# Kuhlman-Lab/ThermoMPNN

Hardware: AMD Instinct MI355X
Metric: mutant ddG preds/sec (SSM, L=256, K=48) (higher is better)
Workload: dtype f32 (per-edge matmuls: f16x2 split on the 16-bit matrix cores, 22 significant bits, fp32 accumulate); 1 GPU; BASELINE configs[1] x 64: 64 synthetic L=256 proteins per GPU (K=48, h=128), full 20xL SSM each, inputs resident in HBM; proteins_per_gpu=64, L=256, K=48, h=128, unit_counted=mutant ddG predictions, weights=synthetic_state_dict(seed=0), parallelism=proteins sharded x1

## Files before the change

### thermompnn_amd/csrc/tmpnn_api.hip

```cpp
#include <stdarg.h>
#include <stdio.h>
#include <stdlib.h>
#include <string.h>

#include <map>
#include <new>
#include <string>
#include <vector>

#include "tmpnn_internal.h"
#include "tmpnn_head_body.h"
#include "../../include/tmpnn_debug.h"

static thread_local char g_err[512] = "";

int tm_set_error(int code, const char *fmt, ...) {
    va_list ap;
    va_start(ap, fmt);
    vsnprintf(g_err, sizeof(g_err), fmt, ap);
    va_end(ap);
    return code;
}
int tm_check_launch(const char *what) {
    hipError_t e = hipGetLastError();
    if (e != hipSuccess) return tm_set_error(TMPNN_E_LAUNCH, "%s: %s", what, hipGetErrorString(e));
    return TMPNN_OK;
}

struct ProfRec { const char *name; hipEvent_t start, stop; };
static bool g_prof_on = false;
static bool g_prof_open = false;
static std::string g_prof_only;
static std::vector<ProfRec> g_prof;
static std::vector<hipEvent_t> g_event_pool;

static hipEvent_t prof_event() {
    if (!g_event_pool.empty()) { hipEvent_t e = g_event_pool.back(); g_event_pool.pop_back(); return e; }
    hipEvent_t e = nullptr;
    if (hipEventCreate(&e) != hipSuccess) return nullptr;
    return e;
}
void tm_prof_begin(const char *name, hipStream_t st) {
    g_prof_open = false;
    if (!g_prof_on || (!g_prof_only.empty() && g_prof_only != name)) return;
    ProfRec r{name, prof_event(), prof_event()};
    if (!r.start || !r.stop) return;
    (void)hipEventRecord(r.start, st);
    g_prof.push_back(r);
    g_prof_open = true;
}
void tm_prof_end(hipStream_t st) {
    if (!g_prof_open) return;
    (void)hipEventRecord(g_prof.back().stop, st);
    g_prof_open = false;
}

extern "C" int tmpnn_profile_select(const char *name) {
    g_prof_only = name ? name : "";
    return TMPNN_OK;
}

extern "C" int tmpnn_profile_enable(int on) {
    for (auto &r : g_prof) { g_event_pool.push_back(r.start); g_event_pool.push_back(r.stop); }
    g_prof.clear();
    g_prof_on = on != 0;
    return TMPNN_OK;
}

extern "C" int tmpnn_profile_fetch(const char **names, double *total_ms, int64_t *launches, int capacity) {
    if (capacity < 0 || (capacity > 0 && (!names || !total_ms || !launches)))
        return tm_set_error(TMPNN_E_INVALID, "profile_fetch: bad arguments");
    std::vector<const char *> order;
    std::map<std::string, std::pair<double, int64_t>> agg;
    for (auto &r : g_prof) {
        if (hipEventSynchronize(r.stop) != hipSuccess) return tm_set_error(TMPNN_E_LAUNCH, "profile_fetch: event sync failed");
        float ms = 0.f;
        if (hipEventElapsedTime(&ms, r.start, r.stop) != hipSuccess) return tm_set_error(TMPNN_E_LAUNCH, "profile_fetch: elapsed failed");
        auto it = agg.find(r.name);
        if (it == agg.end()) { order.push_back(r.name); agg[r.name] = {ms, 1}; }
        else { it->second.first += ms; it->second.second += 1; }
    }
    int n = 0;
    for (const char *nm : order) {
        if (n >= capacity) break;
        names[n] = nm; total_ms[n] = agg[nm].first; launches[n] = agg[nm].second;
        ++n;
    }
    for (auto &r : g_prof) { g_event_pool.push_back(r.start); g_event_pool.push_back(r.stop); }
    g_prof.clear();
    return n;
}
int tm_num_cus() {
    static int cache[64] = {0};
    int dev = 0;
    if (hipGetDevice(&dev) != hipSuccess || dev < 0 || dev >= 64) return 256;
    if (cache[dev] == 0) {
        int n = 0;
        if (hipDeviceGetAttribute(&n, hipDeviceAttributeMultiprocessorCount, dev) != hipSuccess || n <= 0) n = 256;
        cache[dev] = n;
    }
    return cache[dev];
}

static int parse_mode(const char *e) {
    if (e == nullptr || e[0] == 0 || strcmp(e, "f16x2") == 0) return (int)TM_MM_F16X2;
    if (strcmp(e, "bf16x3") == 0) return (int)TM_MM_BF16X3;
    if (strcmp(e, "fp32") == 0) return (int)TM_MM_FP32;
    return -1;
}
static const char *mode_name(int m) { return m == TM_MM_F16X2 ? "f16x2" : m == TM_MM_BF16X3 ? "bf16x3" : "fp32"; }
static int default_mode() {
    static const int v = parse_mode(getenv("TMPNN_PRECISION"));
    return v;
}
extern "C" const char *tmpnn_matmul_mode(void) { return mode_name(default_mode() < 0 ? (int)TM_MM_F16X2 : default_mode()); }
extern "C" const char *tmpnn_weights_precision(const tmpnn_weights_t *w) { return w ? mode_name(w->mode) : nullptr; }

extern "C" int tmpnn_status_error(int32_t status) {
    if (status == 0) return TMPNN_OK;
    if (status & TMPNN_STATUS_MAXLEN)
        return tm_set_error(TMPNN_E_INVALID, "a protein is longer than the max_len passed to the call (its neighbour rows were left empty)");
    if (status & TMPNN_STATUS_RANGE)
        return tm_set_error(TMPNN_E_RANGE, "non-finite ddG / log-probability: an operand left the fp16 range of the f16x2 "
                                           "matrix-core path (|x| >= 65504); use precision \"bf16x3\" (full fp32 range)");
    if (status & TMPNN_STATUS_SELFTEST)
        return tm_set_error(TMPNN_E_UNSUPPORTED, "device self-test failed: this libtmpnn.so was built with flags under which the f16x2 "
                                                 "GELU does not propagate NaN (fp16 overflow would go undetected) or the code-object "
                                                 "ABI differs from v5 (persistent tile loops would stride wrongly); rebuild with "
                                                 "python -m thermompnn_amd.build");
    return tm_set_error(TMPNN_E_INVALID, "unknown status bits 0x%x", (unsigned)status);
}

extern "C" int tmpnn_selftest(int32_t *status, tmpnn_stream_t stream) {
    if (!status) return tm_set_error(TMPNN_E_INVALID, "selftest: null status word");
    return launch_selftest(status, (hipStream_t)stream);
}

extern "C" int tmpnn_version(void) { return TMPNN_VERSION; }
extern "C" const char *tmpnn_last_error(void) { return g_err; }

struct TensorSpec { std::string name; int64_t numel; };

static const std::vector<TensorSpec> &tensor_table() {
    static std::vector<TensorSpec> t;
    if (!t.empty()) return t;
    auto add = [&](const std::string &n, int64_t e) { t.push_back({n, e}); };
    const int H = TMPNN_HID;
    add("features.embeddings.linear.weight", 16 * 66);
    add("features.embeddings.linear.bias", 16);
    add("features.edge_embedding.weight", H * 416);
    add("features.norm_edges.weight", H);
    add("features.norm_edges.bias", H);
    add("W_e.weight", H * H);
    add("W_e.bias", H);
    add("W_s.weight", TMPNN_VOCAB * H);
    auto layer = [&](const std::string &p, int num_in, bool edge) {
        const char *norms[3] = {"norm1", "norm2", "norm3"};
        for (int i = 0; i < (edge ? 3 : 2); ++i) { add(p + "." + norms[i] + ".weight", H); add(p + "." + norms[i] + ".bias", H); }
        add(p + ".W1.weight", (int64_t)H * (H + num_in)); add(p + ".W1.bias", H);
        add(p + ".W2.weight", H * H); add(p + ".W2.bias", H);
        add(p + ".W3.weight", H * H); add(p + ".W3.bias", H);
        if (edge) {
            add(p + ".W11.weight", (int64_t)H * (H + num_in)); add(p + ".W11.bias", H);
            add(p + ".W12.weight", H * H); add(p + ".W12.bias", H);
            add(p + ".W13.weight", H * H); add(p + ".W13.bias", H);
        }
        add(p + ".dense.W_in.weight", 4 * H * H); add(p + ".dense.W_in.bias", 4 * H);
        add(p + ".dense.W_out.weight", 4 * H * H); add(p + ".dense.W_out.bias", H);
    };
    for (int i = 0; i < 3; ++i) layer("encoder_layers." + std::to_string(i), 2 * H, true);
    for (int i = 0; i < 3; ++i) layer("decoder_layers." + std::to_string(i), 3 * H, false);
    add("W_out.weight", TMPNN_VOCAB * H);
    add("W_out.bias", TMPNN_VOCAB);
    add("light_attention.feature_convolution.weight", 384 * 384 * 9);
    add("light_attention.feature_convolution.bias", 384);
    add("light_attention.attention_convolution.weight", 384 * 384 * 9);
    add("light_attention.attention_convolution.bias", 384);
    add("both_out.1.weight", 64 * 384); add("both_out.1.bias", 64);
    add("both_out.3.weight", 32 * 64); add("both_out.3.bias", 32);
    add("both_out.5.weight", TMPNN_VOCAB * 32); add("both_out.5.bias", TMPNN_VOCAB);
    add("ddg_out.weight", 1); add("ddg_out.bias", 1);
    return t;
}

extern "C" int tmpnn_num_tensors(void) { return (int)tensor_table().size(); }
extern "C" const char *tmpnn_tensor_name(int i) {
    const auto &t = tensor_table();
    return (i < 0 || i >= (int)t.size()) ? nullptr : t[i].name.c_str();
}
extern "C" int64_t tmpnn_tensor_numel(int i) {
    const auto &t = tensor_table();
    return (i < 0 || i >= (int)t.size()) ? -1 : t[i].numel;
}

static const size_t POS_TABLE_FLOATS = 66 * TMPNN_HID, SEQ_TABLE_FLOATS = TMPNN_VOCAB * TMPNN_HID,
                    CONV_CENTER_FLOATS = 384 * 384;
static size_t packed_bytes_for(int mode) {
    return (POS_TABLE_FLOATS + 3 * SEQ_TABLE_FLOATS + CONV_CENTER_FLOATS) * sizeof(float) +
           (mode == TM_MM_F16X2 ? (size_t)TM_N_IMG * TM_WIMG_BYTES : 0);
}
extern "C" size_t tmpnn_weights_packed_bytes(void) { return packed_bytes_for(TM_MM_F16X2); }
extern "C" size_t tmpnn_weights_packed_bytes_p(const char *precision) {
    const int mode = precision ? parse_mode(precision) : default_mode();
    return mode < 0 ? 0 : packed_bytes_for(mode);
}

extern "C" int tmpnn_weights_create(tmpnn_weights_t **out, const float *const *tensors, int n_tensors, void *packed,
                                    size_t packed_bytes, tmpnn_stream_t stream) {
    return tmpnn_weights_create_p(out, tensors, n_tensors, packed, packed_bytes, nullptr, stream);
}

extern "C" int tmpnn_weights_create_p(tmpnn_weights_t **out, const float *const *tensors, int n_tensors, void *packed,
                                      size_t packed_bytes, const char *precision, tmpnn_stream_t stream) {
    const int mode = precision ? parse_mode(precision) : default_mode();
    if (mode < 0)
        return tm_set_error(TMPNN_E_INVALID, "weights_create: unknown precision '%s' (f16x2 | bf16x3 | fp32)",
                            precision ? precision : getenv("TMPNN_PRECISION"));
    if (!out || !tensors || !packed) return tm_set_error(TMPNN_E_INVALID, "weights_create: null argument");
    if (tensor_table().size() != TMPNN_N_TENSORS) return tm_set_error(TMPNN_E_INVALID, "internal tensor table size");
    if (n_tensors != TMPNN_N_MPNN_TENSORS && n_tensors != TMPNN_N_TENSORS)
        return tm_set_error(TMPNN_E_INVALID, "weights_create: n_tensors must be %d or %d, got %d", TMPNN_N_MPNN_TENSORS,
                            TMPNN_N_TENSORS, n_tensors);
    if (packed_bytes < packed_bytes_for(mode))
        return tm_set_error(TMPNN_E_WORKSPACE, "weights_create: packed buffer %zu < %zu bytes", packed_bytes,
                            packed_bytes_for(mode));
    if (((uintptr_t)packed & 15) != 0) return tm_set_error(TMPNN_E_INVALID, "weights_create: packed buffer must be 16-byte aligned");
    for (int i = 0; i < n_tensors; ++i)
        if (!tensors[i] || ((uintptr_t)tensors[i] & 15) != 0)
            return tm_set_error(TMPNN_E_INVALID, "weights_create: tensor %d (%s) is null or not 16-byte aligned", i,
                                tmpnn_tensor_name(i));
    tmpnn_weights *w = new (std::nothrow) tmpnn_weights();
    if (!w) return tm_set_error(TMPNN_E_INVALID, "weights_create: host allocation failed");
    memset(w, 0, sizeof(*w));
    w->n_tensors = n_tensors;
    w->mode = mode;
    std::map<std::string, const float *> by_name;
    for (int i = 0; i < n_tensors; ++i) { w->t[i] = tensors[i]; by_name[tensor_table()[i].name] = tensors[i]; }
    auto get = [&](const std::string &n) -> const float * {
        auto it = by_name.find(n);
        return it == by_name.end() ? nullptr : it->second;
    };
    w->pos_w = get("features.embeddings.linear.weight");
    w->pos_b = get("features.embeddings.linear.bias");
    w->edge_w = get("features.edge_embedding.weight");
    w->norm_edges_w = get("features.norm_edges.weight");
    w->norm_edges_b = get("features.norm_edges.bias");
    w->We_w = get("W_e.weight");
    w->We_b = get("W_e.bias");
    w->Ws_w = get("W_s.weight");
    auto node = [&](const std::string &p) {
        return NodeW{get(p + "W3.weight"), get(p + "W3.bias"), get(p + "norm1.weight"), get(p + "norm1.bias"),
                     get(p + "dense.W_in.weight"), get(p + "dense.W_in.bias"), get(p + "dense.W_out.weight"), get(p + "dense.W_out.bias"),
                     get(p + "norm2.weight"), get(p + "norm2.bias"), {}};
    };
    auto proj = [](const float *W, int ld, int c_off, const float *b) {
        return NodeProj{ProjSpec{W, ld, b, W + c_off, ld, nullptr, nullptr, nullptr}, {}};
    };
    for (int l = 0; l < 3; ++l) {
        const std::string p = "encoder_layers." + std::to_string(l) + ".";
        const float *W1 = get(p + "W1.weight"), *W11 = get(p + "W11.weight");
        EncW &e = w->enc[l];
        e.node = node(p);
        e.msg = MsgW{W1 + 128, 384, get(p + "W2.weight"), get(p + "W2.bias"), false, {}};
        e.edge = EdgeW{W11 + 128, get(p + "W12.weight"), get(p + "W12.bias"), get(p + "W13.weight"), get(p + "W13.bias"),
                       get(p + "norm3.weight"), get(p + "norm3.bias"), {}};
        e.msg_proj = proj(W1, 384, 256, get(p + "W1.bias"));
        e.edge_proj = proj(W11, 384, 256, get(p + "W11.bias"));
        const std::string d = "decoder_layers." + std::to_string(l) + ".";
        const float *D1 = get(d + "W1.weight");
        DecW &c = w->dec[l];
        c.node = node(d);
        c.msg = MsgW{D1 + 128, 512, get(d + "W2.weight"), get(d + "W2.bias"), true, {}};
        c.msg_proj = proj(D1, 512, 384, get(d + "W1.bias"));
    }
    w->Wout_w = get("W_out.weight");
    w->Wout_b = get("W_out.bias");
    if (n_tensors == TMPNN_N_TENSORS) {
        w->conv_w = get("light_attention.feature_convolution.weight");
        w->conv_b = get("light_attention.feature_convolution.bias");
        const char *idx[3] = {"1", "3", "5"};
        for (int i = 0; i < 3; ++i) {
            w->mlp_w[i] = get(std::string("both_out.") + idx[i] + ".weight");
            w->mlp_b[i] = get(std::string("both_out.") + idx[i] + ".bias");
        }
        w->ddg_w = get("ddg_out.weight");
        w->ddg_b = get("ddg_out.bias");
    }
    float *p = (float *)packed;
    w->pos_table = p; p += POS_TABLE_FLOATS;
    for (int l = 0; l < 3; ++l) { w->seq_table[l] = p; p += SEQ_TABLE_FLOATS; }
    w->conv_center = p; p += CONV_CENTER_FLOATS;
    int rc = launch_prep_tables(w, (hipStream_t)stream);
    if (mode == TM_MM_F16X2) {
        char *img = (char *)p, *const img_end = img + (size_t)TM_N_IMG * TM_WIMG_BYTES;
        auto image = [&](const float *base, int ld, int n_rows = 128, int k_valid = 128, int k_wrap = 0, bool perm = false) -> const char * {
            if (rc != TMPNN_OK || img == img_end) return nullptr;
            const char *at = img;
            rc = launch_prep_wimg(base, ld, img, (hipStream_t)stream, n_rows, k_valid, k_wrap, perm);
            img += TM_WIMG_BYTES;
            return at;
        };
        auto node_images = [&](NodeW &n) {
            n.img[0] = image(n.W3, 128);
            for (int c = 0; c < 4; ++c) { n.img[1 + 2 * c] = image(n.Win + (size_t)128 * c * 128, 128); n.img[2 + 2 * c] = image(n.Wout + 128 * c, 512); }
        };
        auto proj_images = [&](NodeProj &np) { np.img = {image(np.spec.Wa, np.spec.lda), image(np.spec.Wc, np.spec.ldc)}; };
        auto msg_images = [&](MsgW &m) { m.img.w1 = image(m.W1e, m.ld1); m.img.w2 = image(m.W2, 128); };
        auto msg_images_kperm = [&](MsgW &m) { m.img.p1 = image(m.W1e, m.ld1, 128, 128, 0, true); m.img.p2 = image(m.W2, 128, 128, 128, 0, true); };
        for (int b = 0; b < 4; ++b) w->feat_img.edge[b] = image(w->edge_w + 16 + 128 * b, 416, 128, b < 3 ? 128 : 16, b < 3 ? 0 : 16);
        w->feat_img.we = image(w->We_w, 128);
        if (n_tensors == TMPNN_N_TENSORS) {
            for (int u = 0; u < 9; ++u) w->head_img.unit[u] = image(w->conv_center + (size_t)128 * (u / 3) * 384 + 128 * (u % 3), 384);
            for (int u = 0; u < 3; ++u) w->head_img.unit[9 + u] = image(w->mlp_w[0] + 128 * u, 384, 64);
        }
        for (int l = 0; l < 3; ++l) {
            EncW &e = w->enc[l];
            node_images(e.node); proj_images(e.msg_proj); proj_images(e.edge_proj); msg_images(e.msg);
            e.edge.img = {image(e.edge.W11e, 384), image(e.edge.W12, 128), image(e.edge.W13, 128)};
            DecW &d = w->dec[l];
            node_images(d.node); proj_images(d.msg_proj); msg_images(d.msg);
        }
        for (int l = 0; l < 3; ++l) { msg_images_kperm(w->enc[l].msg); msg_images_kperm(w->dec[l].msg); }
        const int n_built = (int)((img - (char *)p) / TM_WIMG_BYTES), n_want = TM_N_IMG - (n_tensors == TMPNN_N_TENSORS ? 0 : TM_N_HEAD_IMG);
        if (rc == TMPNN_OK && n_built != n_want) rc = tm_set_error(TMPNN_E_INVALID, "weights_create: built %d fragment images, expected %d", n_built, n_want);
    }
    if (rc != TMPNN_OK) { delete w; return rc; }
    *out = w;
    return TMPNN_OK;
}

extern "C" void tmpnn_weights_destroy(tmpnn_weights_t *w) { delete w; }

#define REQUIRE(cond, ...) do { if (!(cond)) return tm_set_error(TMPNN_E_INVALID, __VA_ARGS__); } while (0)
#define TRY(expr) do { int rc_ = (expr); if (rc_ != TMPNN_OK) return rc_; } while (0)

static const int64_t T_MAX = ((int64_t)1 << 31) / (TMPNN_KS * 4) - 1;

static size_t align256(size_t b) { return (b + 255) & ~(size_t)255; }

struct Carver {
    char *p; size_t left;
    void *take(size_t bytes) {
        bytes = align256(bytes);
        if (bytes > left) return nullptr;
        void *r = p; p += bytes; left -= bytes;
        return r;
    }
};

extern "C" size_t tmpnn_layer_workspace_bytes(int64_t T) {
    if (T < 0) return 0;
    return 2 * align256((size_t)T * 256 * 4) + align256((size_t)T * TMPNN_HID * 4) + align256((size_t)T * 4) + 256;
}
extern "C" size_t tmpnn_workspace_bytes(int64_t T) {
    if (T < 0) return 0;
    return tmpnn_layer_workspace_bytes(T) + 2 * align256((size_t)T * TMPNN_KS * 4) +
           align256((size_t)T * TMPNN_KS * TMPNN_HID * 4) + 4 * align256((size_t)T * TMPNN_HID * 4) + 256;
}

static int carve_layer_ws(void *workspace, size_t bytes, int64_t T, LayerWs *ws, Carver *rest = nullptr) {
    uintptr_t base = ((uintptr_t)workspace + 255) & ~(uintptr_t)255;
    size_t skip = base - (uintptr_t)workspace;
    if (!workspace || skip > bytes) return tm_set_error(TMPNN_E_WORKSPACE, "workspace missing or too small");
    Carver c{(char *)base, bytes - skip};
    ws->P = (float *)c.take((size_t)T * 256 * 4);
    ws->P2 = (float *)c.take((size_t)T * 256 * 4);
    ws->Ssum = (float *)c.take((size_t)T * TMPNN_HID * 4);
    ws->cnt = (float *)c.take((size_t)T * 4);
    if (!ws->P || !ws->P2 || !ws->Ssum || !ws->cnt) return tm_set_error(TMPNN_E_WORKSPACE, "workspace too small for T=%lld", (long long)T);
    if (rest) *rest = c;
    return TMPNN_OK;
}

static NodeProj proj_into(NodeProj np, float *P) { np.spec.P = P; return np; }
static NodeProj enc_msg_proj(const tmpnn_weights *w, int l, float *P) { return proj_into(w->enc[l].msg_proj, P); }
static NodeProj enc_edge_proj(const tmpnn_weights *w, int l, float *P) { return proj_into(w->enc[l].edge_proj, P); }
static NodeProj dec_msg_proj(const tmpnn_weights *w, int l, float *P, const int32_t *S) {
    NodeProj np = proj_into(w->dec[l].msg_proj, P);
    if (S) { np.spec.add_tab = w->seq_table[l]; np.spec.add_idx = S; }
    return np;
}

static int run_enc_layer(const tmpnn_weights *w, int l, float *hV, float *hE, const int32_t *E_idx, const float *mask,
                         int64_t T, const LayerWs &ws, bool have_P, bool have_msg, const NodeProj *next, const MsgW *then,
                         hipStream_t st) {
    const EncW &e = w->enc[l];
    if (!have_P) {
        const NodeProj mp = enc_msg_proj(w, l, ws.P);
        TRY(launch_node_proj(hV, mp, T, st));
    }
    if (!have_msg) TRY(launch_msg(w->mode, e.msg, ws.P, hE, E_idx, mask, T, ws.Ssum, ws.cnt, st));
    const NodeProj ep = enc_edge_proj(w, l, ws.P2);
    TRY(launch_node_update(w->mode, e.node, hV, ws.Ssum, ws.cnt, mask, T, hV, &ep, next, st));
    if (then) return launch_edge_msg_fused(e.edge, ws.P2, hE, E_idx, *then, ws.P, mask, T, ws.Ssum, ws.cnt, st);
    return launch_enc_edge(w->mode, e.edge, ws.P2, hE, E_idx, T, st);
}

static int run_dec_layer(const tmpnn_weights *w, int l, const float *hV_in, float *hV_out, const float *hE,
                         const int32_t *E_idx, const int32_t *S, const float *mask, int64_t T, const LayerWs &ws,
                         bool have_P, bool have_msg, const NodeProj *next, hipStream_t st, const HeadArgs *head = nullptr,
                         bool *head_ran = nullptr) {
    const DecW &d = w->dec[l];
    if (!have_P) {
        const NodeProj mp = dec_msg_proj(w, l, ws.P, S);
        TRY(launch_node_proj(hV_in, mp, T, st));
    }
    if (!have_msg) TRY(launch_msg(w->mode, d.msg, ws.P, hE, E_idx, mask, T, ws.Ssum, ws.cnt, st));
    return launch_node_update(w->mode, d.node, hV_in, ws.Ssum, ws.cnt, mask, T, hV_out, next, nullptr, st, head, head_ran);
}

static int run_encoder(const tmpnn_weights *w, const float *X, const float *mask, const int32_t *residue_idx, const int32_t *chain_enc,
                       const int32_t *offsets, int n_proteins, int64_t T, int max_len, int K, const LayerWs &ws, int32_t *E_idx,
                       float *D_nb, float *hE, float *hV, const int32_t *S, float *P_dec0, int32_t *status_opt, bool *dec_msg0_done,
                       hipStream_t st) {
    static const bool fuse_small = TM_DBG_FLAG("TMPNN_FUSE_SMALL", true);
    const KnnInit kinit{hV, ws.P, w->enc[0].msg_proj.spec.ba, status_opt};
    if (fuse_small && max_len <= 256 && featurize_fusable(w->mode, T)) {
        const KnnFuse kf{mask, offsets, n_proteins, max_len, K, E_idx, D_nb, kinit};
        TRY(launch_featurize(w, X, residue_idx, chain_enc, E_idx, D_nb, T, hE, nullptr, st, &kf));
    } else {
        TRY(launch_knn(X, mask, offsets, n_proteins, T, max_len, K, E_idx, D_nb, nullptr, st, kinit));
        TRY(launch_featurize(w, X, residue_idx, chain_enc, E_idx, D_nb, T, hE, nullptr, st));
    }
    const bool fused = fuse_small && edge_msg_fusable(w->mode, T);
    *dec_msg0_done = fused && S;
    for (int l = 0; l < 3; ++l) {
        const NodeProj next = l < 2 ? enc_msg_proj(w, l + 1, ws.P) : dec_msg_proj(w, 0, P_dec0, S);
        const MsgW *then = !fused ? nullptr : l < 2 ? &w->enc[l + 1].msg : S ? &w->dec[0].msg : nullptr;
        TRY(run_enc_layer(w, l, hV, hE, E_idx, mask, T, ws, true, fused && l > 0, &next, then, st));
    }
    return TMPNN_OK;
}

extern "C" int tmpnn_knn_topk(const float *X, const float *mask, const int32_t *offsets, int n_proteins, int64_t T,
                              int max_len, int K, int32_t *E_idx, float *D_nb, int32_t *status_opt, tmpnn_stream_t stream) {
    REQUIRE(X && mask && offsets && E_idx && D_nb, "knn_topk: null pointer");
    REQUIRE(n_proteins >= 0 && T >= 0 && T <= T_MAX, "knn_topk: bad sizes (N=%d, T=%lld)", n_proteins, (long long)T);
    REQUIRE(K >= 1 && K <= TMPNN_KS, "knn_topk: K=%d outside [1, %d]", K, TMPNN_KS);
    if (T == 0 || n_proteins == 0) return TMPNN_OK;
    REQUIRE(max_len >= 1, "knn_topk: max_len must be >= 1");
    if (max_len > 8192) return tm_set_error(TMPNN_E_UNSUPPORTED, "knn_topk: max_len %d > 8192", max_len);
    return launch_knn(X, mask, offsets, n_proteins, T, max_len, K, E_idx, D_nb, status_opt, (hipStream_t)stream);
}

extern "C" int tmpnn_centrality(const float *X, const float *mask, const int32_t *offsets, int n_proteins, int64_t T,
                                float radius, int32_t *out, tmpnn_stream_t stream) {
    REQUIRE(n_proteins >= 0 && T >= 0 && T <= T_MAX && radius > 0.f, "centrality: bad argument");
    if (T == 0 || n_proteins == 0) return TMPNN_OK;
    REQUIRE(X && mask && offsets && out, "centrality: null pointer");
    return launch_centrality(X, mask, offsets, n_proteins, T, radius, out, (hipStream_t)stream);
}

extern "C" int tmpnn_edge_featurize(const tmpnn_weights_t *w, const float *X, const int32_t *residue_idx,
                                    const int32_t *chain_enc, const int32_t *E_idx, const float *D_nb, int64_t T,
                                    float *h_E, float *E_opt, tmpnn_stream_t stream) {
    REQUIRE(w && X && residue_idx && chain_enc && E_idx && D_nb && h_E, "edge_featurize: null pointer");
    REQUIRE(T >= 0 && T <= T_MAX, "edge_featurize: bad T");
    if (T == 0) return TMPNN_OK;
    return launch_featurize(w, X, residue_idx, chain_enc, E_idx, D_nb, T, h_E, E_opt, (hipStream_t)stream);
}

extern "C" int tmpnn_gather_nodes(const float *nodes, const int64_t *neighbor_idx, int B, int N, int K, int C, float *out,
                                  tmpnn_stream_t stream) {
    REQUIRE(B >= 0 && N >= 0 && K >= 0 && C >= 1, "gather_nodes: bad shape");
    if ((int64_t)B * N * K == 0) return TMPNN_OK;
    REQUIRE(nodes && neighbor_idx && out, "gather_nodes: null pointer");
    return launch_gather_rows(nodes, neighbor_idx, 1, (int64_t)B * N * K, (int64_t)N * K, N, C, out, (hipStream_t)stream);
}

extern "C" int tmpnn_gather_rows_i32(const float *nodes, const int32_t *idx, int64_t n_rows, int C, float *out,
                                     tmpnn_stream_t stream) {
    REQUIRE(n_rows >= 0 && C >= 1, "gather_rows_i32: bad shape");
    if (n_rows == 0) return TMPNN_OK;
    REQUIRE(nodes && idx && out, "gather_rows_i32: null pointer");
    return launch_gather_rows(nodes, idx, 0, n_rows, 0, 0, C, out, (hipStream_t)stream);
}

extern "C" int tmpnn_gather_edges(const float *edges, const int64_t *neighbor_idx, int B, int N, int K, int C, float *out,
                                  tmpnn_stream_t stream) {
    REQUIRE(B >= 0 && N >= 0 && K >= 0 && C >= 1, "gather_edges: bad shape");
    if ((int64_t)B * N * K == 0) return TMPNN_OK;
    REQUIRE(edges && neighbor_idx && out, "gather_edges: null pointer");
    return launch_gather_edges(edges, neighbor_idx, B, N, K, C, out, (hipStream_t)stream);
}

extern "C" int tmpnn_enc_layer(const tmpnn_weights_t *w, int layer, float *h_V, float *h_E, const int32_t *E_idx,
                               const float *mask, int64_t T, void *workspace, size_t workspace_bytes,
                               tmpnn_stream_t stream) {
    REQUIRE(w && h_V && h_E && E_idx && mask, "enc_layer: null pointer");
    REQUIRE(layer >= 0 && layer < 3, "enc_layer: layer %d outside [0,3)", layer);
    REQUIRE(T >= 0 && T <= T_MAX, "enc_layer: bad T");
    if (T == 0) return TMPNN_OK;
    LayerWs ws;
    TRY(carve_layer_ws(workspace, workspace_bytes, T, &ws));
    return run_enc_layer(w, layer, h_V, h_E, E_idx, mask, T, ws, false, false, nullptr, nullptr, (hipStream_t)stream);
}

extern "C" int tmpnn_gemm_probe(int mode, const float *X, const float *W, float *Y, int64_t T, int reps, tmpnn_stream_t stream) {
    REQUIRE(X && W && Y && T > 0 && reps > 0 && mode >= 0 && mode <= 2, "gemm_probe: bad argument");
    return launch_gemm_probe(mode, X, W, Y, T, reps, (hipStream_t)stream);
}

extern "C" int tmpnn_clock_probe(int blocks, int iters, uint64_t *out, float *sink, tmpnn_stream_t stream) {
    REQUIRE(blocks > 0 && iters > 0 && out && sink, "clock_probe: bad argument");
    return launch_clock_probe(blocks, iters, (unsigned long long *)out, sink, (hipStream_t)stream);
}

extern "C" int tmpnn_clock_monitor(int iters, uint64_t *out, tmpnn_stream_t stream) {
    REQUIRE(iters > 0 && out, "clock_monitor: bad argument");
    return launch_clock_monitor(iters, (unsigned long long *)out, (hipStream_t)stream);
}

__global__ void launch_probe_kernel(float *buf, int dirty_floats, int k) {
    extern __shared__ float probe_lds[];
    for (int i = blockIdx.x * blockDim.x + threadIdx.x; i < dirty_floats; i += gridDim.x * blockDim.x) buf[i] = (float)k;
    if (dirty_floats < 0) probe_lds[threadIdx.x] = 0.f;
}
extern "C" int tmpnn_launch_probe(int n, int grid, int block, int lds_bytes, float *buf, int dirty_floats, tmpnn_stream_t stream) {
    REQUIRE(n > 0 && grid > 0 && block > 0 && block <= 1024 && lds_bytes >= 0 && lds_bytes <= 160 * 1024, "launch_probe: bad argument");
    REQUIRE(dirty_floats <= 0 || buf, "launch_probe: dirty_floats without a buffer");
    if (lds_bytes > 64 * 1024)
        (void)hipFuncSetAttribute(reinterpret_cast<const void *>(launch_probe_kernel), hipFuncAttributeMaxDynamicSharedMemorySize, 160 * 1024);
    for (int k = 0; k < n; ++k) launch_probe_kernel<<<grid, block, lds_bytes, (hipStream_t)stream>>>(buf, dirty_floats, k);
    return tm_check_launch("launch_probe");
}

extern "C" int tmpnn_dec_layer(const tmpnn_weights_t *w, int layer, const float *h_V_in, float *h_V_out, const float *h_E,
                               const int32_t *E_idx, const int32_t *S, const float *mask, int64_t T, void *workspace,
                               size_t workspace_bytes, tmpnn_stream_t stream) {
    REQUIRE(w && h_V_in && h_V_out && h_E && E_idx && S && mask, "dec_layer: null pointer");
    REQUIRE(layer >= 0 && layer < 3, "dec_layer: layer %d outside [0,3)", layer);
    REQUIRE(T >= 0 && T <= T_MAX, "dec_layer: bad T");
    if (T == 0) return TMPNN_OK;
    LayerWs ws;
    TRY(carve_layer_ws(workspace, workspace_bytes, T, &ws));
    return run_dec_layer(w, layer, h_V_in, h_V_out, h_E, E_idx, S, mask, T, ws, false, false, nullptr, (hipStream_t)stream);
}

extern "C" int tmpnn_seq_embed(const tmpnn_weights_t *w, const int32_t *S, int64_t T, float *h_S, tmpnn_stream_t stream) {
    REQUIRE(w && S && h_S && T >= 0, "seq_embed: bad argument");
    if (T == 0) return TMPNN_OK;
    return launch_seq_embed(w, S, T, h_S, (hipStream_t)stream);
}

extern "C" int tmpnn_log_probs(const tmpnn_weights_t *w, const float *h_V, int64_t T, float *log_probs,
                               int32_t *status_opt, tmpnn_stream_t stream) {
    REQUIRE(w && h_V && log_probs && T >= 0 && T <= T_MAX, "log_probs: bad argument");
    if (T == 0) return TMPNN_OK;
    return launch_log_probs(w, h_V, T, log_probs, status_opt, (hipStream_t)stream);
}

extern "C" int tmpnn_ddg_head(const tmpnn_weights_t *w, const float *hV_last, const float *hV_prev, const int32_t *S,
                              int64_t T, float *ddg, float *z_opt, int32_t *status_opt, tmpnn_stream_t stream) {
    REQUIRE(w && hV_last && hV_prev && S && ddg && T >= 0 && T <= T_MAX, "ddg_head: bad argument");
    REQUIRE(w->n_tensors == TMPNN_N_TENSORS, "ddg_head: weight handle was created without the TransferModel head tensors");
    if (T == 0) return TMPNN_OK;
    return launch_head(w, hV_last, hV_prev, S, T, ddg, z_opt, status_opt, (hipStream_t)stream);
}

static int head_generic_dims_ok(int n_final, int n_layers, const int32_t *dims) {
    if (n_final < 0 || n_final > 3 || n_layers < 1 || n_layers > 8 || !dims) return 0;
    if (dims[0] != TMPNN_HID * n_final + TMPNN_HID || dims[n_layers] != TMPNN_VOCAB) return 0;
    for (int l = 1; l < n_layers; ++l)
        if (dims[l] < 1 || dims[l] > 4096) return 0;
    return 1;
}

extern "C" size_t tmpnn_head_generic_workspace_bytes(int64_t T, int n_final, int n_layers, const int32_t *dims) {
    if (T < 0 || !head_generic_dims_ok(n_final, n_layers, dims)) return 0;
    int widest = dims[0];
    for (int l = 1; l <= n_layers; ++l) widest = dims[l] > widest ? dims[l] : widest;
    return 2 * align256((size_t)T * widest * sizeof(float));
}

extern "C" int tmpnn_ddg_head_generic(const float *const *hidden, int n_final, const float *Ws, const int32_t *S, int64_t T,
                                      const float *conv_w, const float *conv_b, int n_layers, const float *const *mlp_w,
                                      const float *const *mlp_b, const int32_t *dims, const float *ddg_w, const float *ddg_b,
                                      float *ddg, float *z_opt, void *workspace, size_t workspace_bytes, int32_t *status_opt,
                                      tmpnn_stream_t stream) {
    REQUIRE(head_generic_dims_ok(n_final, n_layers, dims),
            "ddg_head_generic: dims must run from 128 * num_final_layers + 128 to 21 over 1..8 layers (num_final_layers 0..3)");
    REQUIRE(Ws && S && mlp_w && mlp_b && ddg_w && ddg_b && ddg && (n_final == 0 || hidden), "ddg_head_generic: null pointer");
    for (int i = 0; i < n_final; ++i) REQUIRE(hidden[i], "ddg_head_generic: hidden[%d] is null", i);
    for (int l = 0; l < n_layers; ++l) REQUIRE(mlp_w[l] && mlp_b[l], "ddg_head_generic: layer %d has a null weight / bias", l);
    REQUIRE((conv_w == nullptr) == (conv_b == nullptr), "ddg_head_generic: conv weight and bias go together");
    REQUIRE(T >= 0 && T <= T_MAX, "ddg_head_generic: bad T");
    if (T == 0) return TMPNN_OK;
    const size_t need = tmpnn_head_generic_workspace_bytes(T, n_final, n_layers, dims);
    if (!workspace || workspace_bytes < need)
        return tm_set_error(TMPNN_E_WORKSPACE, "ddg_head_generic: workspace %zu < %zu bytes", workspace_bytes, need);
    float *buf0 = (float *)workspace, *buf1 = (float *)((char *)workspace + need / 2);
    return launch_head_generic(hidden, n_final, Ws, S, T, conv_w, conv_b, n_layers, mlp_w, mlp_b, dims, ddg_w, ddg_b, ddg, z_opt,
                               buf0, buf1, status_opt, (hipStream_t)stream);
}

extern "C" int tmpnn_ssm_forward(const tmpnn_weights_t *w, const float *X, const int32_t *S, const float *mask,
                                 const int32_t *residue_idx, const int32_t *chain_enc, const int32_t *offsets,
                                 int n_proteins, int64_t T, int max_len, int K, float *ddg, float *hidden_opt,
                                 float *log_probs_opt, int32_t *E_idx_opt, int32_t *status_opt, void *workspace,
                                 size_t workspace_bytes, tmpnn_stream_t stream) {
    REQUIRE(w, "ssm_forward: null weight handle");
    REQUIRE(n_proteins >= 0 && T >= 0 && T <= T_MAX, "ssm_forward: bad sizes");
    REQUIRE(K >= 1 && K <= TMPNN_KS, "ssm_forward: K=%d outside [1, %d]", K, TMPNN_KS);
    REQUIRE(!ddg || w->n_tensors == TMPNN_N_TENSORS, "ssm_forward: ddg requested but the handle has no head tensors");
    if (T == 0 || n_proteins == 0) return TMPNN_OK;
    REQUIRE(X && S && mask && residue_idx && chain_enc && offsets, "ssm_forward: null input pointer");
    REQUIRE(ddg || hidden_opt || log_probs_opt, "ssm_forward: no output requested");
    REQUIRE(max_len >= 1, "ssm_forward: max_len must be >= 1 (the longest protein of the batch)");
    if (max_len > 8192) return tm_set_error(TMPNN_E_UNSUPPORTED, "ssm_forward: max_len %d > 8192", max_len);
    hipStream_t st = (hipStream_t)stream;

    LayerWs ws;
    Carver c{nullptr, 0};
    TRY(carve_layer_ws(workspace, workspace_bytes, T, &ws, &c));
    int32_t *E_idx = (int32_t *)c.take((size_t)T * TMPNN_KS * 4);
    float *D_nb = (float *)c.take((size_t)T * TMPNN_KS * 4);
    float *hE = (float *)c.take((size_t)T * TMPNN_KS * TMPNN_HID * 4);
    float *hV[4];
    for (int i = 0; i < 4; ++i) hV[i] = (float *)c.take((size_t)T * TMPNN_HID * 4);
    if (!E_idx || !D_nb || !hE || !hV[3])
        return tm_set_error(TMPNN_E_WORKSPACE, "ssm_forward: workspace %zu < %zu bytes", workspace_bytes, tmpnn_workspace_bytes(T));
    if (E_idx_opt) E_idx = E_idx_opt;
    if (hidden_opt) for (int l = 0; l < 3; ++l) hV[1 + l] = hidden_opt + (size_t)l * T * TMPNN_HID;

    bool dec_msg0_done = false;
    bool head_done = false;
    TRY(run_encoder(w, X, mask, residue_idx, chain_enc, offsets, n_proteins, T, max_len, K, ws, E_idx, D_nb, hE, hV[0], S, ws.P,
                    status_opt, &dec_msg0_done, st));
    for (int l = 0; l < 3; ++l) {
        const NodeProj next = dec_msg_proj(w, l < 2 ? l + 1 : 2, ws.P, S);
        HeadArgs ha;
        const bool with_head = dec_msg0_done && l == 2 && ddg && node_head_fusable(w->mode, T);
        if (with_head) TRY(tm_head_args(ha, w, hV[3], hV[2], S, T, ddg, nullptr, status_opt, E_idx));
        TRY(run_dec_layer(w, l, hV[l], hV[l + 1], hE, E_idx, S, mask, T, ws, true, dec_msg0_done && l == 0, l < 2 ? &next : nullptr, st,
                          with_head ? &ha : nullptr, with_head ? &head_done : nullptr));
    }
    if (ddg && !head_done) TRY(launch_head(w, hV[3], hV[2], S, T, ddg, nullptr, status_opt, st, E_idx));
    if (log_probs_opt) TRY(launch_log_probs(w, hV[3], T, log_probs_opt, status_opt, st, ddg ? nullptr : E_idx));
    if (!ddg && !log_probs_opt && hidden_opt) TRY(launch_range_check(hV[3], T * TMPNN_HID, status_opt, st, E_idx, T));
    return TMPNN_OK;
}

struct EncCtx { int32_t *E_idx; float *hE, *hV, *P0; };

extern "C" size_t tmpnn_encode_bytes(int64_t T) {
    if (T < 0) return 0;
    return align256((size_t)T * TMPNN_KS * 4) + align256((size_t)T * TMPNN_KS * TMPNN_HID * 4) + align256((size_t)T * TMPNN_HID * 4) +
           align256((size_t)T * 256 * 4);
}
extern "C" size_t tmpnn_encode_workspace_bytes(int64_t T) {
    if (T < 0) return 0;
    return tmpnn_layer_workspace_bytes(T) + align256((size_t)T * TMPNN_KS * 4);
}
extern "C" size_t tmpnn_decode_variants_workspace_bytes(int64_t T, int64_t V) {
    if (T < 0 || V < 0 || (V > 0 && T > T_MAX / V)) return 0;
    const size_t R = (size_t)T * (size_t)V;
    return align256(R * 256 * 4) + 5 * align256(R * TMPNN_HID * 4) + 2 * align256(R * 4) + 256;
}

static int carve_ctx(const char *what, void *ctx, size_t ctx_bytes, int64_t T, EncCtx *c) {
    if (!ctx || ((uintptr_t)ctx & 255) != 0) return tm_set_error(TMPNN_E_INVALID, "%s: ctx is null or not 256-byte aligned", what);
    if (ctx_bytes < tmpnn_encode_bytes(T))
        return tm_set_error(TMPNN_E_WORKSPACE, "%s: ctx %zu < %zu bytes", what, ctx_bytes, tmpnn_encode_bytes(T));
    Carver cv{(char *)ctx, ctx_bytes};
    c->E_idx = (int32_t *)cv.take((size_t)T * TMPNN_KS * 4);
    c->hE = (float *)cv.take((size_t)T * TMPNN_KS * TMPNN_HID * 4);
    c->hV = (float *)cv.take((size_t)T * TMPNN_HID * 4);
    c->P0 = (float *)cv.take((size_t)T * 256 * 4);
    return TMPNN_OK;
}

extern "C" int tmpnn_encode(const tmpnn_weights_t *w, const float *X, const float *mask, const int32_t *residue_idx,
                            const int32_t *chain_enc, const int32_t *offsets, int n_proteins, int64_t T, int max_len, int K,
                            void *ctx, size_t ctx_bytes, int32_t *status_opt, void *workspace, size_t workspace_bytes,
                            tmpnn_stream_t stream) {
    REQUIRE(w, "encode: null weight handle");
    REQUIRE(n_proteins >= 0 && T >= 0 && T <= T_MAX, "encode: bad sizes");
    REQUIRE(K >= 1 && K <= TMPNN_KS, "encode: K=%d outside [1, %d]", K, TMPNN_KS);
    if (T == 0 || n_proteins == 0) return TMPNN_OK;
    REQUIRE(X && mask && residue_idx && chain_enc && offsets, "encode: null input pointer");
    REQUIRE(max_len >= 1, "encode: max_len must be >= 1 (the longest protein of the batch)");
    if (max_len > 8192) return tm_set_error(TMPNN_E_UNSUPPORTED, "encode: max_len %d > 8192", max_len);
    EncCtx c;
    TRY(carve_ctx("encode", ctx, ctx_bytes, T, &c));
    LayerWs ws;
    Carver rest{nullptr, 0};
    TRY(carve_layer_ws(workspace, workspace_bytes, T, &ws, &rest));
    float *D_nb = (float *)rest.take((size_t)T * TMPNN_KS * 4);
    if (!D_nb)
        return tm_set_error(TMPNN_E_WORKSPACE, "encode: workspace %zu < %zu bytes", workspace_bytes, tmpnn_encode_workspace_bytes(T));
    hipStream_t st = (hipStream_t)stream;
    bool unused = false;
    TRY(run_encoder(w, X, mask, residue_idx, chain_enc, offsets, n_proteins, T, max_len, K, ws, c.E_idx, D_nb, c.hE, c.hV, nullptr,
                    c.P0, status_opt, &unused, st));
    return launch_range_check(c.hV, T * TMPNN_HID, status_opt, st, c.E_idx, T);
}

static const int64_t ORD_ROWS_MAX = ((int64_t)1 << 24) - 1;

extern "C" size_t tmpnn_decode_ordered_workspace_bytes(int64_t T, int64_t V) {
    if (T < 0 || V < 0 || (V > 0 && (T > T_MAX / V || T > ORD_ROWS_MAX / (V + 1)))) return 0;
    const size_t R = (size_t)T * (size_t)V;
    return align256((R + (size_t)T) * 256 * 4) + 5 * align256(R * TMPNN_HID * 4) + 2 * align256(R * 4) + align256(R * 8) +
           align256((size_t)T * TMPNN_KS * 4) + 256;
}

static int decode_rows(const char *what, bool ordered, const tmpnn_weights_t *w, const void *ctx, size_t ctx_bytes, const int32_t *S_var,
                       const int32_t *rank, int64_t V, const float *mask, int64_t T, float *ddg, float *hidden_opt, float *log_probs_opt,
                       int32_t *status_opt, void *workspace, size_t workspace_bytes, tmpnn_stream_t stream) {
    REQUIRE(w, "%s: null weight handle", what);
    REQUIRE(T >= 0 && T <= T_MAX && V >= 0, "%s: bad sizes (T=%lld, V=%lld)", what, (long long)T, (long long)V);
    REQUIRE(!ddg || w->n_tensors == TMPNN_N_TENSORS, "%s: ddg requested but the handle has no head tensors", what);
    if (T == 0 || V == 0) return TMPNN_OK;
    if (T > T_MAX / V)
        return tm_set_error(TMPNN_E_UNSUPPORTED, "%s: V * T = %lld * %lld rows exceed %lld (decode the variants in chunks)", what,
                            (long long)V, (long long)T, (long long)T_MAX);
    if (ordered && T > ORD_ROWS_MAX / (V + 1))
        return tm_set_error(TMPNN_E_UNSUPPORTED, "%s: (V + 1) * T = %lld * %lld rows exceed %lld (decode the variants in chunks)", what,
                            (long long)(V + 1), (long long)T, (long long)ORD_ROWS_MAX);
    REQUIRE(S_var && mask && (rank || !ordered), "%s: null input pointer", what);
    REQUIRE(ddg || hidden_opt || log_probs_opt, "%s: no output requested", what);
    EncCtx c;
    TRY(carve_ctx(what, const_cast<void *>(ctx), ctx_bytes, T, &c));
    const int64_t R = V * T;
    const size_t need = ordered ? tmpnn_decode_ordered_workspace_bytes(T, V) : tmpnn_decode_variants_workspace_bytes(T, V);
    uintptr_t base = ((uintptr_t)workspace + 255) & ~(uintptr_t)255;
    if (!workspace || workspace_bytes < need)
        return tm_set_error(TMPNN_E_WORKSPACE, "%s: workspace %zu < %zu bytes", what, workspace_bytes, need);
    Carver cv{(char *)base, workspace_bytes - (base - (uintptr_t)workspace)};
    float *P = (float *)cv.take((size_t)(R + (ordered ? T : 0)) * 256 * 4);
    float *Ssum = (float *)cv.take((size_t)R * TMPNN_HID * 4);
    float *cnt = (float *)cv.take((size_t)R * 4);
    float *mask_rep = (float *)cv.take((size_t)R * 4);
    float *hV[4];
    for (int i = 0; i < 4; ++i) hV[i] = (float *)cv.take((size_t)R * TMPNN_HID * 4);
    void *vis = ordered ? cv.take((size_t)R * 8) : nullptr;
    int32_t *remap = ordered ? (int32_t *)cv.take((size_t)T * TMPNN_KS * 4) : nullptr;
    if (!P || !Ssum || !cnt || !mask_rep || !hV[3] || (ordered && (!vis || !remap)))
        return tm_set_error(TMPNN_E_WORKSPACE, "%s: workspace %zu < %zu bytes", what, workspace_bytes, need);
    hipStream_t st = (hipStream_t)stream;
    float *Penc = P + (size_t)R * 256;
    TRY(launch_variant_expand(c.hV, c.P0, mask, w->seq_table[0], S_var, T, V, hV[0], P, mask_rep, status_opt, st));
    if (ordered) {
        TRY(launch_variant_penc0(c.P0, T, Penc, st));
        TRY(launch_variant_vis(rank, c.E_idx, T, V, vis, st));
    }
    for (int l = 0; l < 3; ++l) {
        TRY(launch_variant_msg(w->mode, w->dec[l].msg, P, c.hE, c.E_idx, mask, T, V, Ssum, cnt, st, vis, remap));
        const NodeProj next = dec_msg_proj(w, l < 2 ? l + 1 : 2, P, S_var);
        TRY(launch_node_update(w->mode, w->dec[l].node, hV[l], Ssum, cnt, mask_rep, R, hV[l + 1], l < 2 ? &next : nullptr, nullptr, st));
        if (ordered && l < 2) {
            const NodeProj pe = dec_msg_proj(w, l + 1, Penc, nullptr);
            TRY(launch_node_proj(c.hV, pe, T, st));
        }
    }
    if (ddg) TRY(launch_head(w, hV[3], hV[2], S_var, R, ddg, nullptr, status_opt, st));
    if (log_probs_opt) TRY(launch_log_probs(w, hV[3], R, log_probs_opt, status_opt, st));
    if (!ddg && !log_probs_opt) TRY(launch_range_check(hV[3], R * TMPNN_HID, status_opt, st));
    if (hidden_opt) TRY(launch_variant_hidden(hV + 1, T, V, hidden_opt, st));
    return TMPNN_OK;
}

extern "C" int tmpnn_decode_variants(const tmpnn_weights_t *w, const void *ctx, size_t ctx_bytes, const int32_t *S_var, int64_t V,
                                     const float *mask, int64_t T, float *ddg, float *hidden_opt, float *log_probs_opt,
                                     int32_t *status_opt, void *workspace, size_t workspace_bytes, tmpnn_stream_t stream) {
    return decode_rows("decode_variants", false, w, ctx, ctx_bytes, S_var, nullptr, V, mask, T, ddg, hidden_opt, log_probs_opt, status_opt,
                       workspace, workspace_bytes, stream);
}

extern "C" int tmpnn_decode_ordered(const tmpnn_weights_t *w, const void *ctx, size_t ctx_bytes, const int32_t *S_var,
                                    const int32_t *rank, int64_t V, const float *mask, int64_t T, float *ddg, float *hidden_opt,
                                    float *log_probs_opt, int32_t *status_opt, void *workspace, size_t workspace_bytes,
                                    tmpnn_stream_t stream) {
    return decode_rows("decode_ordered", true, w, ctx, ctx_bytes, S_var, rank, V, mask, T, ddg, hidden_opt, log_probs_opt, status_opt,
                       workspace, workspace_bytes, stream);
}
```

### thermompnn_amd/csrc/tmpnn_edge.hip

```cpp
#include <stdio.h>
#include <stdlib.h>

#include <type_traits>

#include "tmpnn_split.h"
#include "tmpnn_internal.h"

template <typename SP, bool PROF = false, bool OFF32 = false>
__global__ __launch_bounds__(512, 2) void enc_edge8_rp_kernel(EdgeArgsB a, unsigned long long *prof = nullptr) {
    unsigned t_last = 0, t_acc[11] = {};
    auto mark = [&](int k) {
        if constexpr (PROF) {
            __builtin_amdgcn_sched_barrier(0);
            const unsigned t = (unsigned)__builtin_readcyclecounter();
            if (k >= 0) t_acc[k] += t - t_last;
            t_last = t;
        }
    };
    constexpr int TILEB = SP::NP * SPLIT_PLANE_BYTES;
    __shared__ __attribute__((aligned(16))) char tE[TILEB];
    __shared__ __attribute__((aligned(16))) char tX[TILEB];
    __shared__ __attribute__((aligned(16))) char tY[TILEB];
    __shared__ __attribute__((aligned(16))) float tO[TM_TILE * TM_H];
    __shared__ __attribute__((aligned(16))) float s_par[SP::EXACT ? 4 : 1][TM_H];
    __shared__ __attribute__((aligned(16))) float s_stat[TM_TILE][TM_STAT_LD];
    __shared__ int s_idx[2][TM_TILE];
    const int tid = tm_tid(), lane = tid & 63, wv = tid >> 6, m = lane & 15, q = lane >> 4;

    WFragS<SP> w11[1][4], w12[1][4], w13[1][4];
    load_wfrag_auto<SP>(a.img11, a.W11e, 384, wv, lane, w11[0]);
    load_wfrag_auto<SP>(a.img12, a.W12, TM_H, wv, lane, w12[0]);
    load_wfrag_auto<SP>(a.img13, a.W13, TM_H, wv, lane, w13[0]);
    const int ncol = 16 * wv + 4 * q, c4 = 4 * wv + q;
    const int c32 = lane & 31;
    const unsigned ucol = (unsigned)ncol;
    const unsigned eoff = (unsigned)(m * TM_H + ncol);
    const unsigned soff = (unsigned)((6 * wv + (lane >> 5)) * TM_H + 4 * c32);
    auto prow_of = [&](int j, int self) -> const float * {
        const int jj = j < 0 ? self : j;
        if constexpr (OFF32) return a.P + ((unsigned)jj * 256u + (128u + ucol));
        else return a.P + (size_t)jj * 256 + 128 + ncol;
    };
    constexpr int EPF = SP::EXACT ? 1 : TM_EDGE_PF;
    const f4 z4p = f4{0.f, 0.f, 0.f, 0.f};
    f4 b12r = z4p, b13r = z4p, g4r = z4p, be4r = z4p;
    if constexpr (SP::EXACT) {
        if (tid < 128) st4(&s_par[tid >> 5][4 * (tid & 31)], ld4((tid < 32 ? a.b12 : tid < 64 ? a.b13 : tid < 96 ? a.g3 : a.be3) + 4 * (tid & 31)));
    } else {
        b12r = ld4(a.b12 + ncol); b13r = ld4(a.b13 + ncol);
        g4r = ld4(a.g3 + 4 * c32); be4r = ld4(a.be3 + 4 * c32);
    }
    auto par = [&](int k, int col, const f4 &reg) -> f4 { if constexpr (SP::EXACT) return ld4(&s_par[k][col]); else return reg; };

    const TileRange tr = xcd_tile_range(a.T);
    int i = tr.begin;
    int cur = 0;
    f4 gai, gcj[3], e_cur[3], e_nxt[3];
    if (i < tr.end) {
        if (tid < TM_TILE) s_idx[0][tid] = a.E_idx[(size_t)i * TM_KS + tid];
        const float *src = a.hE + (size_t)i * TM_KS * TM_H;
#pragma unroll
        for (int rb = 0; rb < 3; ++rb) e_cur[rb] = ld4(src + (eoff + 16 * rb * TM_H));
        __syncthreads();
#pragma unroll
        for (int rb = 0; rb < 3; ++rb) store_split<SP>(tE, 16 * rb + m, c4, e_cur[rb]);
        gai = ld4(a.P + (size_t)i * 256 + ucol);
#pragma unroll
        for (int rb = 0; rb < 3; ++rb) gcj[rb] = ld4(prow_of(s_idx[0][16 * rb + m], i));
        touch(gai);
#pragma unroll
        for (int rb = 0; rb < 3; ++rb) touch(gcj[rb]);
        __syncthreads();
    }
    int nidx = -1;
    if (i < tr.end && tid < TM_TILE) nidx = a.E_idx[(size_t)(i + tr.step < tr.end ? i + tr.step : i) * TM_KS + tid];
    mark(-1);
    unsigned long long c_begin = 0, w_begin = 0;
    if (PROF) { c_begin = __builtin_readcyclecounter(); w_begin = wall_clock64(); }
    for (; i < tr.end; i += tr.step) {
        float *tile_g = a.hE + (size_t)i * TM_KS * TM_H;
        const int inext = i + tr.step;
        const bool has_next = inext < tr.end;
        const int ipf = has_next ? inext : i;
        const int ipf2 = ipf + tr.step < tr.end ? ipf + tr.step : ipf;
        const int nidx_pub = nidx;
        const float *src = a.hE + (size_t)ipf * TM_KS * TM_H;
        f4 acc[3][1];
#pragma unroll
        for (int rb = 0; rb < 3; ++rb) acc[rb][0] = gai + gcj[rb];
        mma_tile_split_ride<SP, 4, 3, EPF>(tE, w11, acc, lane, [&](auto S) {
            constexpr int s = decltype(S)::value;
            if constexpr (s == 1) { if (tid < TM_TILE) nidx = a.E_idx[(size_t)ipf2 * TM_KS + tid]; }
#if TM_ABL_NOLOAD
            if constexpr (s % 3 == 0 && s >= 3) e_nxt[s / 3 - 1] = e_cur[s / 3 - 1];
#else
            if constexpr (!SP::EXACT && s % 3 == 0 && s >= 3) e_nxt[s / 3 - 1] = ld4(src + (eoff + 16 * (s / 3 - 1) * TM_H));
#endif
        });
        mark(0);
        {
            f4 g[3];
#pragma unroll
            for (int rb = 0; rb < 3; ++rb) g[rb] = gelu4(acc[rb][0]);
            __builtin_amdgcn_sched_barrier(0);
#pragma unroll
            for (int rb = 0; rb < 3; ++rb) store_split<SP>(tX, 16 * rb + m, c4, g[rb]);
        }
        if (tid < TM_TILE) s_idx[cur ^ 1][tid] = nidx_pub;
        mark(1);
        __syncthreads();
        mark(2);

#pragma unroll
        for (int rb = 0; rb < 3; ++rb) acc[rb][0] = par(0, ncol, b12r);
        mma_tile_split_ride<SP, 4, 3, EPF>(tX, w12, acc, lane, [&](auto S) {
            constexpr int s = decltype(S)::value;
            if constexpr (SP::EXACT) {
                if constexpr (s % 3 == 0 && s >= 3) e_nxt[s / 3 - 1] = ld4(src + (eoff + 16 * (s / 3 - 1) * TM_H));
            } else {
                if constexpr (s == 1) gai = ld4(a.P + (size_t)ipf * 256 + ucol);
                if constexpr (s % 3 == 0 && s >= 3) gcj[s / 3 - 1] = ld4(prow_of(s_idx[cur ^ 1][16 * (s / 3 - 1) + m], ipf));
            }
        });
        mark(3);
        {
            f4 g[3];
#pragma unroll
            for (int rb = 0; rb < 3; ++rb) g[rb] = gelu4(acc[rb][0]);
            __builtin_amdgcn_sched_barrier(0);
#pragma unroll
            for (int rb = 0; rb < 3; ++rb) store_split<SP>(tY, 16 * rb + m, c4, g[rb]);
        }
        mark(4);
        __syncthreads();
        mark(5);

#pragma unroll
        for (int rb = 0; rb < 3; ++rb) acc[rb][0] = par(1, ncol, b13r);
        mma_tile_split<SP, 4, 1, 3, TM_TILE, 256, 4, 0, true, EPF>(tY, w13, acc, lane);
        if constexpr (SP::EXACT) {
            gai = ld4(a.P + (size_t)ipf * 256 + ucol);
#pragma unroll
            for (int rb = 0; rb < 3; ++rb) gcj[rb] = ld4(prow_of(s_idx[cur ^ 1][16 * rb + m], ipf));
        }
        mark(6);
#pragma unroll
        for (int rb = 0; rb < 3; ++rb) {
            f4 v;
            if constexpr (SP::EXACT) v = load_joined<SP>(tE, 16 * rb + m, c4) + acc[rb][0];
            else v = e_cur[rb] + acc[rb][0];
            st4(tO + chunk_off(16 * rb + m, c4), v);
#if TM_ABL_NOLN
            (void)q;
#else
            row_stats_partial16(v, &s_stat[16 * rb + m][2 * wv], q);
#endif
            store_split<SP>(tE, 16 * rb + m, c4, e_nxt[rb]);
            e_cur[rb] = e_nxt[rb];
        }
        bool okr[3];
#pragma unroll
        for (int it = 0; it < 3; ++it) okr[it] = s_idx[cur][6 * wv + 2 * it + (lane >> 5)] >= 0;
        mark(7);
        __syncthreads();
        mark(8);

        touch(gai);
#pragma unroll
        for (int rb = 0; rb < 3; ++rb) touch(gcj[rb]);
#pragma unroll
        for (int it = 0; it < 3; ++it) {
            const int row = 6 * wv + 2 * it + (lane >> 5);
            float mean = 0.f, rstd = 1.f;
#if !TM_ABL_NOLN
            row_stats_finish8d(&s_stat[row][0], lane, mean, rstd);
#endif
            const f4 x4 = ld4(tO + chunk_off(row, c32));
            const f4 g4 = par(2, 4 * c32, g4r), be4 = par(3, 4 * c32, be4r);
            const f2 s01 = f2{g4.x, g4.y} * rstd, s23 = f2{g4.z, g4.w} * rstd;
            const f2 t01 = __builtin_elementwise_fma(f2{-mean, -mean}, s01, f2{be4.x, be4.y});
            const f2 t23 = __builtin_elementwise_fma(f2{-mean, -mean}, s23, f2{be4.z, be4.w});
            const f2 y01 = __builtin_elementwise_fma(f2{x4.x, x4.y}, s01, t01), y23 = __builtin_elementwise_fma(f2{x4.z, x4.w}, s23, t23);
            const f4 y = f4{y01.x, y01.y, y23.x, y23.y};
            st4(tile_g + (soff + 2 * it * TM_H), okr[it] ? y : f4{0.f, 0.f, 0.f, 0.f});
        }
        cur ^= 1;
        mark(9);
        mark(10);
    }
    if (PROF && tm_bid() == 0 && tm_tid() == TM_PROF_TID) {
#pragma unroll
        for (int k = 0; k < 11; ++k) prof[k] = t_acc[k];
        prof[11] = __builtin_readcyclecounter() - c_begin;
        prof[12] = wall_clock64() - w_begin;
    }
}

int launch_enc_edge_split(int mode, const EdgeW &e, const float *P, float *hE, const int32_t *E_idx, int64_t T, hipStream_t st) {
    const bool h2 = mode == TM_MM_F16X2;
    EdgeArgsB a{e.W11e, e.W12, e.b12, e.W13, e.b13, e.n3w, e.n3b, P, hE, E_idx, (int)T, e.img.w11, e.img.w12, e.img.w13};
    if (h2 && !(a.img11 && a.img12 && a.img13))
        return tm_set_error(TMPNN_E_INVALID, "enc_edge_split: f16x2 handle without the fragment images of W11e / W12 / W13");
    const int64_t cap = tm_num_cus();
    const int grid = (int)(T < cap ? T : cap);
    if (mode == TM_MM_BF16X3) {
        if (T < ((int64_t)1 << 22)) enc_edge8_rp_kernel<SplitBF3, false, true><<<grid, 512, 0, st>>>(a);
        else enc_edge8_rp_kernel<SplitBF3><<<grid, 512, 0, st>>>(a);
    }
    else {
#ifdef TMPNN_DEBUG_BUILD
        static const bool prof = TM_DBG_FLAG("TMPNN_EDGE_PROF", false);
#else
        constexpr bool prof = false;
#endif
        if (prof) {
#ifdef TMPNN_DEBUG_BUILD
            static unsigned long long *d_prof = nullptr;
            if (!d_prof) (void)hipMalloc(&d_prof, 16 * sizeof(unsigned long long));
            (void)hipMemsetAsync(d_prof, 0, 16 * sizeof(unsigned long long), st);
            enc_edge8_rp_kernel<SplitH2, true, false><<<grid, 512, 0, st>>>(a, d_prof);
            unsigned long long h[16];
            (void)hipMemcpy(h, d_prof, sizeof(h), hipMemcpyDeviceToHost);
            const long long tiles0 = T >= 8 * cap ? (T / 8 + cap / 8 - 1) / (cap / 8) : (T + cap - 1) / cap;
            fprintf(stderr, "enc_edge phases (cycles, wg 0): gemm1 %llu gelu+split %llu bar %llu gather+gemm2 %llu gelu+split %llu bar %llu gemm3 %llu resid+stats %llu bar %llu split+ln+store %llu bar %llu; loop %llu cycles in %llu ticks of 100 MHz = %.3f GHz, %lld tiles = %.0f cycles per tile\n",
                    h[0], h[1], h[2], h[3], h[4], h[5], h[6], h[7], h[8], h[9], h[10], h[11], h[12], h[12] ? h[11] / (h[12] * 10.0) : 0.0,
                    tiles0, tiles0 ? (double)h[11] / tiles0 : 0.0);
#endif
        } else if (T < ((int64_t)1 << 22)) {
            enc_edge8_rp_kernel<SplitH2, false, true><<<grid, 512, 0, st>>>(a);
        } else {
            enc_edge8_rp_kernel<SplitH2><<<grid, 512, 0, st>>>(a);
        }
    }
    return tm_check_launch("enc_edge_split");
}
```

### thermompnn_amd/csrc/tmpnn_internal.h

```cpp
#pragma once
#include <hip/hip_runtime.h>
#include <stdint.h>

#include "../../include/tmpnn.h"

#define TM_WIMG_BYTES 65536
#define TM_IMG_COUNT(S) ((int)(sizeof(S::img) / sizeof(const char *)))

struct ProjSpec { const float *Wa; int lda; const float *ba; const float *Wc; int ldc; float *P; const float *add_tab; const int32_t *add_idx; };
struct NodeProj { ProjSpec spec; struct { const char *a, *c; } img; };
struct NodeW {
    const float *W3, *b3, *n1w, *n1b, *Win, *bin, *Wout, *bout, *n2w, *n2b;
    const char *img[9];
};
struct MsgW {
    const float *W1e; int ld1; const float *W2, *b2;
    bool dec;
    struct { const char *w1, *w2, *p1, *p2; } img;
};
struct EdgeW {
    const float *W11e, *W12, *b12, *W13, *b13, *n3w, *n3b;
    struct { const char *w11, *w12, *w13; } img;
};
struct EncW { NodeW node; MsgW msg; EdgeW edge; NodeProj msg_proj, edge_proj; };
struct DecW { NodeW node; MsgW msg; NodeProj msg_proj; };
struct FeatImg { const char *edge[4], *we; };
struct HeadImg { const char *unit[12]; };

struct tmpnn_weights {
    int n_tensors;
    int mode;
    const float *t[TMPNN_N_TENSORS];
    const float *pos_w, *pos_b, *edge_w, *norm_edges_w, *norm_edges_b, *We_w, *We_b, *Ws_w;
    FeatImg feat_img;
    EncW enc[3];
    DecW dec[3];
    const float *Wout_w, *Wout_b;
    const float *conv_w, *conv_b, *mlp_w[3], *mlp_b[3], *ddg_w, *ddg_b;
    HeadImg head_img;
    float *pos_table;
    float *seq_table[3];
    float *conv_center;
};
enum {
    TM_N_ENC_IMG = TM_IMG_COUNT(NodeW) + TM_IMG_COUNT(MsgW) + TM_IMG_COUNT(EdgeW) + 2 * TM_IMG_COUNT(NodeProj),
    TM_N_DEC_IMG = TM_IMG_COUNT(NodeW) + TM_IMG_COUNT(MsgW) + TM_IMG_COUNT(NodeProj),
    TM_N_HEAD_IMG = (int)(sizeof(HeadImg) / sizeof(const char *)),
    TM_N_IMG = (int)(sizeof(FeatImg) / sizeof(const char *)) + TM_N_HEAD_IMG + 3 * TM_N_ENC_IMG + 3 * TM_N_DEC_IMG
};
static_assert(TM_N_IMG == 122, "tmpnn_weights_packed_bytes() is part of the ABI: 122 images of 64 KB + the tables");

struct LayerWs {
    float *P;
    float *P2;
    float *Ssum;
    float *cnt;
};

int tm_set_error(int code, const char *fmt, ...);
int tm_check_launch(const char *what);
void tm_prof_begin(const char *name, hipStream_t st);
void tm_prof_end(hipStream_t st);

struct KnnInit { float *hV0; float *P; const float *ba; int32_t *status_zero; };
int launch_knn(const float *X, const float *mask, const int32_t *offsets, int N, int64_t T, int max_len, int K,
               int32_t *E_idx, float *D_nb, int32_t *status, hipStream_t st, KnnInit init = KnnInit{nullptr, nullptr, nullptr, nullptr});
int launch_centrality(const float *X, const float *mask, const int32_t *offsets, int N, int64_t T, float radius,
                      int32_t *out, hipStream_t st);
struct KnnFuse { const float *mask; const int32_t *offsets; int N, max_len, K; int32_t *E_idx; float *D_nb; KnnInit init; };
bool featurize_fusable(int mode, int64_t T);
int launch_featurize(const tmpnn_weights *w, const float *X, const int32_t *ridx, const int32_t *cenc,
                     const int32_t *E_idx, const float *D_nb, int64_t T, float *h_E, float *E_opt, hipStream_t st,
                     const KnnFuse *knn = nullptr);
int launch_gather_rows(const float *nodes, const void *idx, int idx64, int64_t n_rows, int64_t rows_per_batch,
                       int64_t nodes_per_batch, int C, float *out, hipStream_t st);
int launch_gather_edges(const float *edges, const int64_t *idx, int B, int N, int K, int C, float *out, hipStream_t st);

int launch_msg(int mode, const MsgW &m, const float *P, const float *hE, const int32_t *E_idx, const float *mask, int64_t T,
               float *Ssum, float *cnt, hipStream_t st);
struct NodeArgs {
    const float *W3, *b3, *n1w, *n1b, *Win, *bin, *Wout, *bout, *n2w, *n2b;
    const float *h_in, *Ssum, *cnt, *mask;
    float *h_out;
    int T;
    ProjSpec proj[2];
    const char *img[13];
};
struct HeadArgs;
int launch_node_update_split(const NodeArgs &a, int64_t T, hipStream_t st, const HeadArgs *head = nullptr, bool *head_ran = nullptr);
bool node_head_fusable(int mode, int64_t T);
int launch_node_proj(const float *h, const NodeProj &np, int64_t T, hipStream_t st);
int launch_node_update(int mode, const NodeW &n, const float *h_in, const float *Ssum, const float *cnt, const float *mask, int64_t T,
                       float *h_out, const NodeProj *p0, const NodeProj *p1, hipStream_t st, const HeadArgs *head = nullptr,
                       bool *head_ran = nullptr);
int launch_enc_edge(int mode, const EdgeW &e, const float *P, float *hE, const int32_t *E_idx, int64_t T, hipStream_t st);

int launch_head(const tmpnn_weights *w, const float *hA, const float *hB, const int32_t *S, int64_t T, float *ddg,
                float *z_opt, int32_t *status, hipStream_t st, const int32_t *maxlen_probe = nullptr);
int tm_head_args(HeadArgs &a, const tmpnn_weights *w, const float *hA, const float *hB, const int32_t *S, int64_t T, float *ddg,
                 float *z_opt, int32_t *status, const int32_t *maxlen_probe);
int launch_log_probs(const tmpnn_weights *w, const float *h, int64_t T, float *out, int32_t *status, hipStream_t st,
                     const int32_t *maxlen_probe = nullptr);
int launch_seq_embed(const tmpnn_weights *w, const int32_t *S, int64_t T, float *hS, hipStream_t st);
int launch_head_generic(const float *const *hidden, int n_final, const float *Ws, const int32_t *S, int64_t T, const float *conv_w,
                        const float *conv_b, int n_layers, const float *const *mlp_w, const float *const *mlp_b, const int32_t *dims,
                        const float *ddg_w, const float *ddg_b, float *ddg, float *z_opt, float *buf0, float *buf1, int32_t *status,
                        hipStream_t st);
int tm_head_train_core(const float *feat, int64_t n_feat, const int32_t *rows, const int32_t *mut, const int32_t *wt,
                       const float *target, int64_t M, int lightattn, int n_layers, const int32_t *dims, int subtract_mut,
                       const float *params, float *grads, float p_drop, const float *keep_in, float *keep_out, uint64_t seed,
                       uint64_t step, float *loss, float *pred_opt, void *workspace, hipStream_t st, float *dfeat,
                       const float *dpred);
int tm_head_forward(const float *feat, int64_t n_feat, const int32_t *rows, const int32_t *mut, const int32_t *wt, int64_t M,
                    int lightattn, int n_layers, const int32_t *dims, int subtract_mut, const float *params, float p_drop,
                    const float *keep_in, float *keep_out, uint64_t seed, uint64_t step, float *pred, void *workspace, hipStream_t st);
int launch_range_check(const float *x, int64_t n, int32_t *status, hipStream_t st, const int32_t *maxlen_probe = nullptr,
                       int64_t T = 0);
int launch_prep_tables(tmpnn_weights *w, hipStream_t st);

int launch_clock_probe(int blocks, int iters, unsigned long long *out, float *sink, hipStream_t st);
int launch_clock_monitor(int iters, unsigned long long *out, hipStream_t st);
int launch_enc_edge_split(int mode, const EdgeW &e, const float *P, float *hE, const int32_t *E_idx, int64_t T, hipStream_t st);
int launch_msg_split(int mode, const MsgW &m, const float *P, const float *hE, const int32_t *E_idx, const float *mask, int64_t T,
                     float *Ssum, float *cnt, hipStream_t st);
int launch_gemm_probe(int mode, const float *X, const float *W, float *Y, int64_t T, int reps, hipStream_t st);
bool edge_msg_fusable(int mode, int64_t T);
int launch_edge_msg_fused(const EdgeW &e, const float *P_edge, float *hE, const int32_t *E_idx, const MsgW &m, const float *P_msg,
                          const float *mask, int64_t T, float *Ssum, float *cnt, hipStream_t st);
int launch_variant_expand(const float *hV, const float *P0, const float *mask, const float *tab, const int32_t *S_var, int64_t T,
                          int64_t V, float *hV_rep, float *P, float *mask_rep, int32_t *status, hipStream_t st);
int launch_variant_msg(int mode, const MsgW &m, const float *P, const float *hE, const int32_t *E_idx, const float *mask, int64_t T,
                       int64_t V, float *Ssum, float *cnt, hipStream_t st, const void *vis = nullptr, int32_t *remap = nullptr);
int launch_variant_vis(const int32_t *rank, const int32_t *E_idx, int64_t T, int64_t V, void *vis, hipStream_t st);
int launch_variant_penc0(const float *P0, int64_t T, float *Penc, hipStream_t st);
int launch_variant_hidden(const float *const *h, int64_t T, int64_t V, float *out, hipStream_t st);
int launch_selftest(int32_t *status, hipStream_t st);
int tm_num_cus();
#ifdef TMPNN_DEBUG_BUILD
#include <stdlib.h>
#define TM_DBG_FLAG(name, dflt) ([] { const char *e_ = getenv(name); return e_ ? e_[0] != '0' : (bool)(dflt); }())
#define TM_DBG_INT(name, dflt) ([] { const char *e_ = getenv(name); return e_ ? atoi(e_) : (int)(dflt); }())
#else
#define TM_DBG_FLAG(name, dflt) ((bool)(dflt))
#define TM_DBG_INT(name, dflt) ((int)(dflt))
#endif
enum { TM_MM_FP32 = 0, TM_MM_BF16X3 = 1, TM_MM_F16X2 = 2 };
int launch_prep_wimg(const float *W, int ld, char *dst, hipStream_t st, int n_rows = 128, int k_valid = 128, int k_wrap = 0, bool perm = false);
__device__ __forceinline__ bool tm_nonfinite_bits(unsigned b) { return (b & 0x7f800000u) == 0x7f800000u; }
__device__ __forceinline__ bool tm_nonfinite(float x) { return tm_nonfinite_bits(__float_as_uint(x)); }
__device__ __forceinline__ bool tm_f16_range_bits(unsigned b) { return (b & 0x7fffffffu) >= 0x477fe000u; }
__device__ __forceinline__ bool tm_f16_range_computed(float x) {
    asm volatile("" : "+v"(x));
    return tm_f16_range_bits(__float_as_uint(x));
}
```

### thermompnn_amd/csrc/tmpnn_layers.hip

```cpp
#include <stdlib.h>

#include "tmpnn_common.h"
#include "tmpnn_internal.h"

__global__ __launch_bounds__(TM_THREADS, 2) void node_proj_kernel(const float *__restrict__ h,
                                                                  const float *__restrict__ Wa, int lda,
                                                                  const float *__restrict__ ba,
                                                                  const float *__restrict__ Wc, int ldc, int T,
                                                                  float *__restrict__ P,
                                                                  const float *__restrict__ add_tab,
                                                                  const int32_t *__restrict__ add_idx) {
    __shared__ __attribute__((aligned(16))) float tA[TM_TILE * TM_H];
    const int tid = tm_tid(), lane = tid & 63, wv = tid >> 6, m = lane & 15, q = lane >> 4;
    float wa[2][32], wc[2][32];
    f4 bias[2];
#pragma unroll
    for (int cb = 0; cb < 2; ++cb) {
        const int n0 = 32 * wv + 16 * cb;
        load_wfrag<8>(Wa, lda, n0, 0, TM_H, wa[cb], lane);
        load_wfrag<8>(Wc, ldc, n0, 0, TM_H, wc[cb], lane);
        bias[cb] = ld4(ba + n0 + 4 * q);
    }
    const int n_tiles = (T + TM_TILE - 1) / TM_TILE;
    for (int tile = tm_bid(); tile < n_tiles; tile += tm_nblk()) {
        const int r0 = tile * TM_TILE;
        load_tile(tA, h + (size_t)r0 * TM_H, min(TM_TILE, T - r0), tid);
        __syncthreads();
        f4 acc[3][2];
#pragma unroll
        for (int half = 0; half < 2; ++half) {
#pragma unroll
            for (int rb = 0; rb < 3; ++rb)
#pragma unroll
                for (int cb = 0; cb < 2; ++cb) acc[rb][cb] = half ? f4{0.f, 0.f, 0.f, 0.f} : bias[cb];
            if (half) mma_tile<8, 2>(tA, wc, acc, lane);
            else mma_tile<8, 2>(tA, wa, acc, lane);
#pragma unroll
            for (int rb = 0; rb < 3; ++rb) {
                const int row = r0 + 16 * rb + m;
                if (row < T) {
                    const float *add = half && add_tab ? add_tab + add_idx[row] * TM_H : nullptr;
#pragma unroll
                    for (int cb = 0; cb < 2; ++cb) {
                        const int n = 32 * wv + 16 * cb + 4 * q;
                        st4(P + (size_t)row * 256 + 128 * half + n, add ? ld4(add + n) + acc[rb][cb] : acc[rb][cb]);
                    }
                }
            }
        }
        __syncthreads();
    }
}

struct MsgArgs {
    const float *W1e; int ld1;
    const float *W2, *b2;
    const float *P;
    const float *hE;
    const int32_t *E_idx;
    const float *mask;
    float *Ssum, *cnt;
    int T;
    int skew;
};

template <bool DEC, int NW>
__global__ __launch_bounds__(64 * NW, NW / 2) void msg_kernel(MsgArgs a) {
    constexpr int NT = 64 * NW, NCB = 8 / NW;
    __shared__ __attribute__((aligned(16))) float tE[TM_TILE * TM_H];
    __shared__ __attribute__((aligned(16))) float tA[TM_TILE * TM_H];
    __shared__ float s_part[3][TM_H];
    __shared__ int s_idx[TM_TILE];
    __shared__ float s_ma[TM_TILE];
    const int tid = tm_tid(), lane = tid & 63, wv = tid >> 6, m = lane & 15, q = lane >> 4;
    const int col0 = (TM_H / NW) * wv, chunk0 = (32 / NW) * wv;

    float w1[NCB][32], w2[NCB][32];
    f4 bias2[NCB];
#pragma unroll
    for (int cb = 0; cb < NCB; ++cb) {
        const int n0 = col0 + 16 * cb;
        load_wfrag<8>(a.W1e, a.ld1, n0, 0, TM_H, w1[cb], lane);
        load_wfrag<8>(a.W2, TM_H, n0, 0, TM_H, w2[cb], lane);
        bias2[cb] = ld4(a.b2 + n0 + 4 * q);
    }

    const TileRange tr = xcd_tile_range(a.T);
    for (int i = tr.begin; i < tr.end; i += tr.step) {
        const float mi = a.mask[i];
        if (tid < TM_TILE) {
            const int j = a.E_idx[(size_t)i * TM_KS + tid];
            s_idx[tid] = j;
            s_ma[tid] = j < 0 ? 0.f : (DEC ? 1.f : mi * a.mask[j]);
        }
        load_tile_async<NW>(tE, a.hE + (size_t)i * TM_KS * TM_H, wv, lane);
        __syncthreads();

        f4 acc[3][NCB];
        int jrow[3];
#pragma unroll
        for (int rb = 0; rb < 3; ++rb) {
            const int j = s_idx[16 * rb + m];
            jrow[rb] = j < 0 ? i : j;
        }
#pragma unroll
        for (int cb = 0; cb < NCB; ++cb) {
            const int n = col0 + 16 * cb + 4 * q;
            if (DEC) {
#pragma unroll
                for (int rb = 0; rb < 3; ++rb)
                    acc[rb][cb] = ld4(a.P + (size_t)jrow[rb] * 256 + 128 + n);
            } else {
                const f4 ai = ld4(a.P + (size_t)i * 256 + n);
#pragma unroll
                for (int rb = 0; rb < 3; ++rb) acc[rb][cb] = ai + ld4(a.P + (size_t)jrow[rb] * 256 + 128 + n);
            }
        }
        mma_tile<8, NCB>(tE, w1, acc, lane);
#pragma unroll
        for (int cb = 0; cb < NCB; ++cb) {
            const int n = col0 + 16 * cb + 4 * q;
            f4 ai;
            if (DEC) ai = ld4(a.P + (size_t)i * 256 + n);
#pragma unroll
            for (int rb = 0; rb < 3; ++rb) {
                f4 v = acc[rb][cb];
                if (DEC) v = ai + mi * v;
                st4(tA + chunk_off(16 * rb + m, chunk0 + 4 * cb + q), gelu4(v));
            }
        }
        __syncthreads();

#pragma unroll
        for (int rb = 0; rb < 3; ++rb)
#pragma unroll
            for (int cb = 0; cb < NCB; ++cb) acc[rb][cb] = bias2[cb];
        mma_tile<8, NCB>(tA, w2, acc, lane);
#pragma unroll
        for (int rb = 0; rb < 3; ++rb) {
            const float ma = s_ma[16 * rb + m];
#pragma unroll
            for (int cb = 0; cb < NCB; ++cb) {
                f4 v = gelu4(acc[rb][cb]) * ma;
                if (ma == 0.f) v = f4{0.f, 0.f, 0.f, 0.f};
                st4(tE + chunk_off(16 * rb + m, chunk0 + 4 * cb + q), v);
            }
        }
        __syncthreads();

        {
            constexpr int G = NT / TM_H, RPG = TM_TILE / G;
            const int n = tid & 127, grp = tid >> 7;
            float s = 0.f;
#pragma unroll 8
            for (int r = RPG * grp; r < RPG * grp + RPG; ++r) s += tE[chunk_off(r, n >> 2) + (n & 3)];
            if (grp) s_part[grp - 1][n] = s;
            __syncthreads();
            if (!grp) {
#pragma unroll
                for (int g = 0; g < G - 1; ++g) s += s_part[g][n];
                a.Ssum[(size_t)i * TM_H + n] = s;
            }
            if (tid == 128) {
                float c = 0.f;
                for (int r = 0; r < TM_TILE; ++r) c += s_ma[r];
                a.cnt[i] = c;
            }
        }
        __syncthreads();
    }
}

struct EdgeArgs {
    const float *W11e;
    const float *W12, *b12, *W13, *b13, *g3, *be3;
    const float *P;
    float *hE;
    const int32_t *E_idx;
    int T;
};

__device__ __forceinline__ void row_stats_partial1(const f4 v, float *stat_slot, int q) {
    float mean = (v.x + v.y + v.z + v.w) * 0.25f;
    const f4 d = v - mean;
    float m2 = d.x * d.x + d.y * d.y + d.z * d.z + d.w * d.w;
    float n = 4.f;
#pragma unroll
    for (int off = 16; off <= 32; off <<= 1) {
        const float mo = __shfl_xor(mean, off), m2o = __shfl_xor(m2, off);
        const float delta = mo - mean;
        mean = 0.5f * (mean + mo);
        m2 = m2 + m2o + delta * delta * (0.5f * n);
        n *= 2.f;
    }
    if (q == 0) { stat_slot[0] = mean; stat_slot[1] = m2; }
}
__device__ __forceinline__ void row_stats_finish8(const float *stat_row , float &mean, float &rstd) {
    f4 p[4];
#pragma unroll
    for (int k = 0; k < 4; ++k) p[k] = ld4(stat_row + 4 * k);
    mean = 0.125f * (p[0].x + p[0].z + p[1].x + p[1].z + p[2].x + p[2].z + p[3].x + p[3].z);
    float m2 = 0.f, dd = 0.f;
#pragma unroll
    for (int k = 0; k < 4; ++k) {
        const float d0 = p[k].x - mean, d1 = p[k].z - mean;
        m2 += p[k].y + p[k].w;
        dd += d0 * d0 + d1 * d1;
    }
    rstd = 1.0f / sqrtf((m2 + 16.f * dd) * (1.0f / 128.0f) + 1e-5f);
}

__global__ __launch_bounds__(512, 2) void enc_edge8_kernel(EdgeArgs a) {
    __shared__ __attribute__((aligned(16))) float tE[2][TM_TILE * TM_H];
    __shared__ __attribute__((aligned(16))) float tA[TM_TILE * TM_H];
    __shared__ __attribute__((aligned(16))) float tB[TM_TILE * TM_H];
    __shared__ __attribute__((aligned(16))) float s_stat[TM_TILE][16];
    __shared__ int s_idx[2][TM_TILE];
    const int tid = tm_tid(), lane = tid & 63, wv = tid >> 6, m = lane & 15, q = lane >> 4;

    float w11[1][32], w12[1][32], w13[1][32];
    load_wfrag<8>(a.W11e, 384, 16 * wv, 0, TM_H, w11[0], lane);
    load_wfrag<8>(a.W12, TM_H, 16 * wv, 0, TM_H, w12[0], lane);
    load_wfrag<8>(a.W13, TM_H, 16 * wv, 0, TM_H, w13[0], lane);
    const int ncol = 16 * wv + 4 * q, chunk = 4 * wv + q;
    const f4 b12 = ld4(a.b12 + ncol), b13 = ld4(a.b13 + ncol);
    const int c32 = lane & 31;
    const f4 g4 = ld4(a.g3 + 4 * c32), be4 = ld4(a.be3 + 4 * c32);

    const TileRange tr = xcd_tile_range(a.T);
    int i = tr.begin;
    int cur = 0;
    f4 gai, gcj[3];
    if (i < tr.end) {
        if (tid < TM_TILE) s_idx[0][tid] = a.E_idx[(size_t)i * TM_KS + tid];
        load_tile_async<8>(tE[0], a.hE + (size_t)i * TM_KS * TM_H, wv, lane);
        __syncthreads();
        gai = ld4(a.P + (size_t)i * 256 + ncol);
#pragma unroll
        for (int rb = 0; rb < 3; ++rb) {
            const int j = s_idx[0][16 * rb + m];
            gcj[rb] = ld4(a.P + (size_t)(j < 0 ? i : j) * 256 + 128 + ncol);
        }
    }
    for (; i < tr.end; i += tr.step) {
        float *tile_g = a.hE + (size_t)i * TM_KS * TM_H;
        const float *tEc = tE[cur];
        const int inext = i + tr.step;
        const bool has_next = inext < tr.end;
        int nidx = -1;
        if (has_next) {
            load_tile_async<8>(tE[cur ^ 1], a.hE + (size_t)inext * TM_KS * TM_H, wv, lane);
            if (tid < TM_TILE) nidx = a.E_idx[(size_t)inext * TM_KS + tid];
        }
        f4 acc[3][1];
#pragma unroll
        for (int rb = 0; rb < 3; ++rb) acc[rb][0] = gai + gcj[rb];
        mma_tile<8, 1>(tEc, w11, acc, lane);
#pragma unroll
        for (int rb = 0; rb < 3; ++rb) st4(tA + chunk_off(16 * rb + m, chunk), gelu4(acc[rb][0]));
        if (has_next && tid < TM_TILE) s_idx[cur ^ 1][tid] = nidx;
        __syncthreads();

        if (has_next) {
            gai = ld4(a.P + (size_t)inext * 256 + ncol);
#pragma unroll
            for (int rb = 0; rb < 3; ++rb) {
                const int j = s_idx[cur ^ 1][16 * rb + m];
                gcj[rb] = ld4(a.P + (size_t)(j < 0 ? inext : j) * 256 + 128 + ncol);
            }
        }
#pragma unroll
        for (int rb = 0; rb < 3; ++rb) acc[rb][0] = b12;
        mma_tile<8, 1>(tA, w12, acc, lane);
#pragma unroll
        for (int rb = 0; rb < 3; ++rb) st4(tB + chunk_off(16 * rb + m, chunk), gelu4(acc[rb][0]));
        __syncthreads();

#pragma unroll
        for (int rb = 0; rb < 3; ++rb) acc[rb][0] = b13;
        mma_tile<8, 1>(tB, w13, acc, lane);
#pragma unroll
        for (int rb = 0; rb < 3; ++rb) {
            const int off = chunk_off(16 * rb + m, chunk);
            const f4 v = ld4(tEc + off) + acc[rb][0];
            st4(tA + off, v);
            row_stats_partial1(v, &s_stat[16 * rb + m][2 * wv], q);
        }
        __syncthreads();

#pragma unroll
        for (int it = 0; it < 3; ++it) {
            const int row = 6 * wv + 2 * it + (lane >> 5);
            float mean, rstd;
            row_stats_finish8(&s_stat[row][0], mean, rstd);
            const f4 y = (ld4(tA + chunk_off(row, c32)) - mean) * rstd * g4 + be4;
            if (s_idx[cur][row] >= 0) st4(tile_g + (size_t)row * TM_H + 4 * c32, y);
        }
        cur ^= 1;
        __syncthreads();
    }
}


template <int NRB>
__global__ __launch_bounds__(TM_THREADS, 2) void node_update_kernel(NodeArgs a) {
    constexpr int ROWS = 16 * NRB;
    __shared__ __attribute__((aligned(16))) float tA[ROWS * TM_H];
    __shared__ __attribute__((aligned(16))) float tB[ROWS * TM_H];
    const int tid = tm_tid(), lane = tid & 63, wv = tid >> 6, m = lane & 15, q = lane >> 4;
    const int c32 = lane & 31;
    const int n_tiles = (a.T + ROWS - 1) / ROWS;

    for (int tile = tm_bid(); tile < n_tiles; tile += tm_nblk()) {
        const int r0 = tile * ROWS;
        load_tile<NRB>(tA, a.Ssum + (size_t)r0 * TM_H, min(ROWS, a.T - r0), tid);
        __syncthreads();

        float wf[2][32];
        f4 acc[NRB][2];
#pragma unroll
        for (int cb = 0; cb < 2; ++cb) load_wfrag<8>(a.W3, TM_H, 32 * wv + 16 * cb, 0, TM_H, wf[cb], lane);
#pragma unroll
        for (int rb = 0; rb < NRB; ++rb)
#pragma unroll
            for (int cb = 0; cb < 2; ++cb) acc[rb][cb] = f4{0.f, 0.f, 0.f, 0.f};
        mma_tile<8, 2, 128, NRB>(tA, wf, acc, lane);
#pragma unroll
        for (int rb = 0; rb < NRB; ++rb) {
            const int row = r0 + 16 * rb + m;
            const bool ok = row < a.T;
            const float c = ok ? a.cnt[row] : 0.f;
#pragma unroll
            for (int cb = 0; cb < 2; ++cb) {
                const int n = 32 * wv + 16 * cb + 4 * q;
                const f4 hv = ok ? ld4(a.h_in + (size_t)row * TM_H + n) : f4{0.f, 0.f, 0.f, 0.f};
                const f4 dh = (acc[rb][cb] + c * ld4(a.b3 + n)) / 30.0f;
                st4(tB + chunk_off(16 * rb + m, 8 * wv + 4 * cb + q), hv + dh);
            }
        }
        __syncthreads();
        {
            const f4 g4 = ld4(a.n1w + 4 * c32), b4 = ld4(a.n1b + 4 * c32);
#pragma unroll
            for (int it = 0; it < 2 * NRB; ++it) {
                const int row = 4 * NRB * wv + 2 * it + (lane >> 5);
                float *p = tB + chunk_off(row, c32);
                st4(p, layer_norm_row(ld4(p), g4, b4));
            }
        }
        __syncthreads();

        f4 out[NRB][2];
#pragma unroll
        for (int cb = 0; cb < 2; ++cb) {
            const f4 b = ld4(a.bout + 32 * wv + 16 * cb + 4 * q);
#pragma unroll
            for (int rb = 0; rb < NRB; ++rb) out[rb][cb] = b;
        }
        for (int c = 0; c < 4; ++c) {
#pragma unroll
            for (int cb = 0; cb < 2; ++cb) {
                const int n0 = 128 * c + 32 * wv + 16 * cb;
                load_wfrag<8>(a.Win, TM_H, n0, 0, 512, wf[cb], lane);
                const f4 b = ld4(a.bin + n0 + 4 * q);
#pragma unroll
                for (int rb = 0; rb < NRB; ++rb) acc[rb][cb] = b;
            }
            mma_tile<8, 2, 128, NRB>(tB, wf, acc, lane);
#pragma unroll
            for (int rb = 0; rb < NRB; ++rb)
#pragma unroll
                for (int cb = 0; cb < 2; ++cb)
                    st4(tA + chunk_off(16 * rb + m, 8 * wv + 4 * cb + q), gelu4(acc[rb][cb]));
            __syncthreads();
#pragma unroll
            for (int cb = 0; cb < 2; ++cb) load_wfrag<8>(a.Wout, 512, 32 * wv + 16 * cb, 128 * c, TM_H, wf[cb], lane);
            mma_tile<8, 2, 128, NRB>(tA, wf, out, lane);
            __syncthreads();
        }
#pragma unroll
        for (int rb = 0; rb < NRB; ++rb)
#pragma unroll
            for (int cb = 0; cb < 2; ++cb) {
                const int off = chunk_off(16 * rb + m, 8 * wv + 4 * cb + q);
                st4(tA + off, ld4(tB + off) + out[rb][cb]);
            }
        __syncthreads();
        {
            const f4 g4 = ld4(a.n2w + 4 * c32), b4 = ld4(a.n2b + 4 * c32);
#pragma unroll
            for (int it = 0; it < 2 * NRB; ++it) {
                const int row = 4 * NRB * wv + 2 * it + (lane >> 5);
                const int grow = r0 + row;
                f4 y = layer_norm_row(ld4(tA + chunk_off(row, c32)), g4, b4);
                y = grow < a.T ? y * a.mask[grow] : f4{0.f, 0.f, 0.f, 0.f};
                st4(tB + chunk_off(row, c32), y);
                if (grow < a.T) st4(a.h_out + (size_t)grow * TM_H + 4 * c32, y);
            }
        }
        __syncthreads();
#pragma unroll
        for (int k = 0; k < 2; ++k) {
            const ProjSpec &ps = a.proj[k];
            if (ps.P == nullptr) continue;
#pragma unroll
            for (int half = 0; half < 2; ++half) {
#pragma unroll
                for (int cb = 0; cb < 2; ++cb) {
                    const int n0 = 32 * wv + 16 * cb;
                    if (half) load_wfrag<8>(ps.Wc, ps.ldc, n0, 0, TM_H, wf[cb], lane);
                    else load_wfrag<8>(ps.Wa, ps.lda, n0, 0, TM_H, wf[cb], lane);
                    const f4 b = half ? f4{0.f, 0.f, 0.f, 0.f} : ld4(ps.ba + n0 + 4 * q);
#pragma unroll
                    for (int rb = 0; rb < NRB; ++rb) acc[rb][cb] = b;
                }
                mma_tile<8, 2, 128, NRB>(tB, wf, acc, lane);
#pragma unroll
                for (int rb = 0; rb < NRB; ++rb) {
                    const int row = r0 + 16 * rb + m;
                    if (row < a.T) {
                        const float *add = half && ps.add_tab ? ps.add_tab + ps.add_idx[row] * TM_H : nullptr;
#pragma unroll
                        for (int cb = 0; cb < 2; ++cb) {
                            const int n = 32 * wv + 16 * cb + 4 * q;
                            st4(ps.P + (size_t)row * 256 + 128 * half + n, add ? ld4(add + n) + acc[rb][cb] : acc[rb][cb]);
                        }
                    }
                }
            }
        }
        __syncthreads();
    }
}

static int grid_for(int64_t work_items, int blocks_per_cu) {
    const int64_t cap = (int64_t)tm_num_cus() * blocks_per_cu;
    return (int)(work_items < cap ? (work_items < 1 ? 1 : work_items) : cap);
}

int launch_node_proj(const float *h, const NodeProj &np, int64_t T, hipStream_t st) {
    const int64_t tiles = (T + TM_TILE - 1) / TM_TILE;
    { tm_prof_begin("node_proj", st); node_proj_kernel<<<grid_for(tiles, 2), TM_THREADS, 0, st>>>(h, np.spec.Wa, np.spec.lda, np.spec.ba, np.spec.Wc, np.spec.ldc, (int)T, np.spec.P, np.spec.add_tab, np.spec.add_idx); tm_prof_end(st); }
    return tm_check_launch("node_proj");
}

int launch_msg(int mode, const MsgW &m, const float *P, const float *hE, const int32_t *E_idx, const float *mask, int64_t T,
               float *Ssum, float *cnt, hipStream_t st) {
    const bool dec = m.dec;
    tm_prof_begin(dec ? "dec_msg" : "enc_msg", st);
    if (mode != TM_MM_FP32) {
        const int rc = launch_msg_split(mode, m, P, hE, E_idx, mask, T, Ssum, cnt, st);
        tm_prof_end(st);
        return rc;
    }
    MsgArgs a{m.W1e, m.ld1, m.W2, m.b2, P, hE, E_idx, mask, Ssum, cnt, (int)T, 0};
    if (dec) msg_kernel<true, 4><<<grid_for(T, 2), 256, 0, st>>>(a);
    else msg_kernel<false, 4><<<grid_for(T, 2), 256, 0, st>>>(a);
    tm_prof_end(st);
    return tm_check_launch(dec ? "dec_msg" : "enc_msg");
}

int launch_enc_edge(int mode, const EdgeW &e, const float *P, float *hE, const int32_t *E_idx, int64_t T, hipStream_t st) {
    tm_prof_begin("enc_edge", st);
    if (mode != TM_MM_FP32) {
        const int rc = launch_enc_edge_split(mode, e, P, hE, E_idx, T, st);
        tm_prof_end(st);
        return rc;
    }
    EdgeArgs a{e.W11e, e.W12, e.b12, e.W13, e.b13, e.n3w, e.n3b, P, hE, E_idx, (int)T};
    enc_edge8_kernel<<<grid_for(T, 1), 512, 0, st>>>(a);
    tm_prof_end(st);
    return tm_check_launch("enc_edge8");
}

int launch_node_update(int mode, const NodeW &n, const float *h_in, const float *Ssum, const float *cnt, const float *mask, int64_t T,
                       float *h_out, const NodeProj *p0, const NodeProj *p1, hipStream_t st, const HeadArgs *head, bool *head_ran) {
    if (head_ran) *head_ran = false;
    NodeArgs a{n.W3, n.b3, n.n1w, n.n1b, n.Win, n.bin, n.Wout, n.bout, n.n2w, n.n2b, h_in, Ssum, cnt, mask, h_out, (int)T, {}, {}};
    const NodeProj *ps[2] = {p0, p1};
    for (int k = 0; k < 2; ++k)
        if (ps[k]) a.proj[k] = ps[k]->spec;
    if (mode == TM_MM_F16X2) {
        for (int u = 0; u < 9; ++u) a.img[u] = n.img[u];
        for (int k = 0; k < 2; ++k)
            if (ps[k]) { a.img[9 + 2 * k] = ps[k]->img.a; a.img[10 + 2 * k] = ps[k]->img.c; }
        for (int u = 0; u < 13; ++u)
            if ((u < 9 || ps[(u - 9) / 2]) && !a.img[u])
                return tm_set_error(TMPNN_E_INVALID, "node_update: f16x2 handle without the fragment image of unit %d", u);
        tm_prof_begin("node_update", st);
        const int rc = launch_node_update_split(a, T, st, head, head_ran);
        tm_prof_end(st);
        return rc;
    }
    tm_prof_begin("node_update", st);
    const int64_t slots = (int64_t)2 * tm_num_cus();
    int best_rows = 48;
    int64_t best_cost = -1;
    for (int rows = 48; rows >= 16; rows -= 16) {
        const int64_t tiles = (T + rows - 1) / rows, rounds = (tiles + slots - 1) / slots;
        const int64_t cost = rounds * (rows + 16);
        if (best_cost < 0 || cost < best_cost) { best_cost = cost; best_rows = rows; }
    }
    const int64_t tiles = (T + best_rows - 1) / best_rows;
    if (best_rows == 16) node_update_kernel<1><<<grid_for(tiles, 2), TM_THREADS, 0, st>>>(a);
    else if (best_rows == 32) node_update_kernel<2><<<grid_for(tiles, 2), TM_THREADS, 0, st>>>(a);
    else node_update_kernel<3><<<grid_for(tiles, 2), TM_THREADS, 0, st>>>(a);
    tm_prof_end(st);
    return tm_check_launch("node_update");
}

__global__ __launch_bounds__(TM_THREADS, 1) void clock_probe_kernel(int iters, unsigned long long *out, float *sink) {
    __shared__ __attribute__((aligned(16))) float tile[TM_TILE * TM_H];
    const int tid = tm_tid(), lane = tid & 63;
    for (int k = tid; k < TM_TILE * TM_H; k += TM_THREADS) tile[k] = 1e-3f * (float)(k & 255);
    float w[2][32];
#pragma unroll
    for (int k = 0; k < 32; ++k) { w[0][k] = 1e-3f * (float)(k + lane); w[1][k] = 1e-3f * (float)(k - lane); }
    f4 acc[3][2];
#pragma unroll
    for (int rb = 0; rb < 3; ++rb)
#pragma unroll
        for (int cb = 0; cb < 2; ++cb) acc[rb][cb] = f4{0.f, 0.f, 0.f, 0.f};
    __syncthreads();
    const unsigned long long c0 = __builtin_readcyclecounter(), t0 = wall_clock64();
    for (int it = 0; it < iters; ++it) mma_tile<8, 2>(tile, w, acc, lane);
    const unsigned long long c1 = __builtin_readcyclecounter(), t1 = wall_clock64();
    float sum = 0.f;
#pragma unroll
    for (int rb = 0; rb < 3; ++rb)
#pragma unroll
        for (int cb = 0; cb < 2; ++cb) sum += acc[rb][cb].x + acc[rb][cb].w;
    if (sum == 123.456f) sink[tid] = sum;
    if (tid == 0) { out[2 * tm_bid()] = c1 - c0; out[2 * tm_bid() + 1] = t1 - t0; }
}

int launch_clock_probe(int blocks, int iters, unsigned long long *out, float *sink, hipStream_t st) {
    clock_probe_kernel<<<blocks, TM_THREADS, 0, st>>>(iters, out, sink);
    return tm_check_launch("clock_probe");
}

__global__ void clock_monitor_kernel(int iters, unsigned long long *out) {
    const unsigned long long c0 = __builtin_readcyclecounter(), t0 = wall_clock64();
    for (int it = 0; it < iters; ++it) __builtin_amdgcn_s_sleep(127);
    const unsigned long long c1 = __builtin_readcyclecounter(), t1 = wall_clock64();
    if (tm_tid() == 0) { out[0] = c1 - c0; out[1] = t1 - t0; }
}
int launch_clock_monitor(int iters, unsigned long long *out, hipStream_t st) {
    clock_monitor_kernel<<<1, 64, 0, st>>>(iters, out);
    return tm_check_launch("clock_monitor");
}
```

### thermompnn_amd/csrc/tmpnn_msg.hip

```cpp
#include <stdio.h>
#include <stdlib.h>

#include <type_traits>

#include "tmpnn_split.h"
#include "tmpnn_internal.h"

template <typename SP, bool DEC, bool PROF = false, bool OFF32 = false>
__global__ __launch_bounds__(512, 2) void msg8_rp_kernel(MsgArgsB a, unsigned long long *prof = nullptr) {
    unsigned long long t_last = 0;
    auto mark = [&](int k) {
        if (PROF && tm_bid() == 0 && tm_tid() == TM_PROF_TID) {
            const unsigned long long t = __builtin_readcyclecounter();
            if (k >= 0) prof[k] += t - t_last;
            t_last = t;
        }
    };
    constexpr int TILEB = SP::NP * SPLIT_PLANE_BYTES;
    __shared__ __attribute__((aligned(16))) char tE[TILEB];
    __shared__ __attribute__((aligned(16))) char tA[TILEB];
    __shared__ int s_idx[2][TM_TILE];
    __shared__ float s_ma[2][TM_TILE];
    const int tid = tm_tid(), lane = tid & 63, wv = tid >> 6, m = lane & 15, q = lane >> 4;

    constexpr bool PERM = SP::NP == 2;
    WFragS<SP> w1[1][4], w2[1][4];
    load_wfrag_auto<SP, PERM>(PERM ? a.imgp1 : a.img1, a.W1e, a.ld1, wv, lane, w1[0]);
    load_wfrag_auto<SP, PERM>(PERM ? a.imgp2 : a.img2, a.W2, TM_H, wv, lane, w2[0]);
    const int ncol = 16 * wv + 4 * q, c4 = 4 * wv + q;
    const int c4s = PERM ? perm_c4(c4) : c4;
    const f4 bias2 = ld4(a.b2 + ncol);

    auto stage_idx = [&](int ii, int buf) {
        if (tid < TM_TILE) {
            const int j = (a.E_idx + (size_t)__builtin_amdgcn_readfirstlane(ii) * TM_KS)[(unsigned)tid];
            s_idx[buf][tid] = j;
            s_ma[buf][tid] = j < 0 ? 0.f : (DEC ? 1.f : a.mask[ii] * a.mask[j]);
        }
    };
    f4 g0, gj[3], e_nxt[3];
    const unsigned ucol = (unsigned)ncol;
    auto gather = [&](int ii, int buf) {
        g0 = ld4(a.P + (size_t)__builtin_amdgcn_readfirstlane(ii) * 256 + ucol);
#pragma unroll
        for (int rb = 0; rb < 3; ++rb) {
            const int j0 = s_idx[buf][16 * rb + m];
            const int j = j0 < 0 ? ii : j0;
            if constexpr (OFF32) gj[rb] = ld4(a.P + ((unsigned)j * 256u + (128u + ucol)));
            else gj[rb] = ld4(a.P + (size_t)j * 256 + 128 + ncol);
        }
    };
    const int prow = 6 * wv + (lane >> 5), pc = lane & 31;
    const int pcs = PERM ? perm_c4(pc) : pc;
    const unsigned eoff = (unsigned)(prow * TM_H + 4 * pc);
    auto fetch_into = [&](f4 (&dst)[3], int ii) {
        const float *src = a.hE + (size_t)__builtin_amdgcn_readfirstlane(ii) * (TM_KS * TM_H);
#pragma unroll
        for (int it = 0; it < 3; ++it) dst[it] = ld4(src + (eoff + 2 * it * TM_H));
    };
    auto fetch_tile = [&](int ii) { fetch_into(e_nxt, ii); };
    auto split_tile = [&]() {
#pragma unroll
        for (int it = 0; it < 3; ++it) store_split<SP>(tE, prow + 2 * it, pcs, e_nxt[it]);
    };

    TileRange tr = xcd_tile_range(a.T);
    tr.begin += a.i0;
    tr.end += a.i0;
    int i = tr.begin;
    int cur = 0;
    if (i < tr.end) {
        stage_idx(i, 0);
        fetch_tile(i);
        __syncthreads();
        split_tile();
        gather(i, 0);
        fetch_tile(i + tr.step < tr.end ? i + tr.step : i);
        __syncthreads();
    }
    float mi = i < tr.end ? a.mask[i] : 0.f;
    mark(-1);
    for (; i < tr.end; i += tr.step) {
        const int inext = i + tr.step;
        const int ipf = inext < tr.end ? inext : i;
        int nidx = -1;
        if (tid < TM_TILE) nidx = (a.E_idx + (size_t)__builtin_amdgcn_readfirstlane(ipf) * TM_KS)[(unsigned)tid];
        const float mi_nxt = (a.mask + __builtin_amdgcn_readfirstlane(ipf))[0];
        f4 acc[3][1];
#pragma unroll
        for (int rb = 0; rb < 3; ++rb) acc[rb][0] = DEC ? gj[rb] : g0 + gj[rb];
        mma_tile_split<SP, 4, 1, 3, TM_TILE, 256, 4, 0, true, TM_MSG_PF>(tE, w1, acc, lane);
        mark(0);
        float mk_j = 1.f;
        if (!DEC && tid < TM_TILE) mk_j = a.mask[(unsigned)(nidx >= 0 ? nidx : ipf)];
#pragma unroll
        for (int rb = 0; rb < 3; ++rb) {
            f4 v = acc[rb][0];
            if (DEC) v = g0 + mi * v;
            store_split<SP>(tA, 16 * rb + m, c4s, gelu4(v));
        }
        if (tid < TM_TILE) {
            s_idx[cur ^ 1][tid] = nidx;
            s_ma[cur ^ 1][tid] = nidx >= 0 ? (DEC ? 1.f : mi_nxt * mk_j) : 0.f;
        }
        mark(1);
        __syncthreads();
        mark(2);

        split_tile();
        const int ipf3 = ipf + tr.step < tr.end ? ipf + tr.step : ipf;
        const float *src3 = a.hE + (size_t)__builtin_amdgcn_readfirstlane(ipf3) * (TM_KS * TM_H);
        mark(3);
#pragma unroll
        for (int rb = 0; rb < 3; ++rb) acc[rb][0] = bias2;
        mma_tile_split_ride<SP, 4, 3, TM_MSG_PF>(tA, w2, acc, lane, [&](auto S) {
            constexpr int s = decltype(S)::value;
            if constexpr (s == 0) g0 = ld4(a.P + (size_t)__builtin_amdgcn_readfirstlane(ipf) * 256 + ucol);
            if constexpr (s >= 1 && s <= 3) {
                const int j0 = s_idx[cur ^ 1][16 * (s - 1) + m];
                const int j = j0 < 0 ? ipf : j0;
                if constexpr (OFF32) gj[s - 1] = ld4(a.P + ((unsigned)j * 256u + (128u + ucol)));
                else gj[s - 1] = ld4(a.P + (size_t)j * 256 + 128 + ncol);
            }
#if !TM_ABL_NOLOAD
            if constexpr (s >= 5 && s <= 9 && (s & 1)) e_nxt[(s - 5) >> 1] = ld4(src3 + (eoff + 2 * ((s - 5) >> 1) * TM_H));
#endif
        });
        mark(4);
        f4 tot = f4{0.f, 0.f, 0.f, 0.f};
#pragma unroll
        for (int rb = 0; rb < 3; ++rb) {
            const float ma = s_ma[cur][16 * rb + m];
            const f4 g = gelu4(acc[rb][0]);
            tot = f4{__builtin_fmaf(g.x, ma, tot.x), __builtin_fmaf(g.y, ma, tot.y), __builtin_fmaf(g.z, ma, tot.z), __builtin_fmaf(g.w, ma, tot.w)};
        }
#pragma unroll
        for (int c = 0; c < 4; ++c) {
            float x = tot[c];
            x += __int_as_float(__builtin_amdgcn_update_dpp(0, __float_as_int(x), 0x111, 0xf, 0xf, true));
            x += __int_as_float(__builtin_amdgcn_update_dpp(0, __float_as_int(x), 0x112, 0xf, 0xf, true));
            x += __int_as_float(__builtin_amdgcn_update_dpp(0, __float_as_int(x), 0x114, 0xf, 0xf, true));
            x += __int_as_float(__builtin_amdgcn_update_dpp(0, __float_as_int(x), 0x118, 0xf, 0xf, true));
            tot[c] = x;
        }
        {
            touch(g0);
#pragma unroll
            for (int rb = 0; rb < 3; ++rb) touch(gj[rb]);
        }
        if (m == 15) st4(a.Ssum + (size_t)__builtin_amdgcn_readfirstlane(i) * TM_H + ucol, tot);
        if (wv == 2) {
            float c = lane < TM_TILE ? s_ma[cur][lane] : 0.f;
#define TM_DPP_ADD(ctrl, row_mask, bc)                                                                  \
            c += __int_as_float(__builtin_amdgcn_update_dpp(0, __float_as_int(c), ctrl, row_mask, 0xf, bc));
            TM_DPP_ADD(0x111, 0xf, true)
            TM_DPP_ADD(0x112, 0xf, true)
            TM_DPP_ADD(0x114, 0xf, true)
            TM_DPP_ADD(0x118, 0xf, true)
            TM_DPP_ADD(0x142, 0xa, false)
            TM_DPP_ADD(0x143, 0xc, false)
#undef TM_DPP_ADD
            if (lane == 63) a.cnt[i] = c;
        }
        mark(5);
        mark(6);
        cur ^= 1;
        mi = mi_nxt;
        __syncthreads();
        mark(7);
    }
}

#define TM_MSG_WAVE_MIN 2
#define TM_MSG_WAVE_ILV 2

template <typename R>
__device__ __forceinline__ void mma_wave_lds(const char *wl, const u4 (&x)[4][2], f4 (&acc)[8], R &&ride) {
    constexpr int NS = 32, ILV = TM_MSG_WAVE_ILV, NG = NS / ILV;
    u4 w[2][ILV][2];
#if TM_ABL_NOMFMA
    static_for<0, NG>([&](auto G) { ride(G); });
    return;
#endif
    auto request = [&](int g, int half) {
#if defined(TM_ABL_WAVE_NOLDS)
        if (g > 1) return;
#endif
#pragma unroll
        for (int k = 0; k < ILV; ++k) {
            const int s = g * ILV + k;
            w[half][k][0] = *reinterpret_cast<const u4 *>(wl + (s & 7) * 8192 + (s >> 3) * 2048);
            w[half][k][1] = *reinterpret_cast<const u4 *>(wl + (s & 7) * 8192 + (s >> 3) * 2048 + 1024);
        }
    };
    request(0, 0);
#define TM_HF(a, b, c) __builtin_amdgcn_mfma_f32_16x16x32_f16(__builtin_bit_cast(h8, a), __builtin_bit_cast(h8, b), c, 0, 0, 0)
    static_for<0, NG>([&](auto G) {
        constexpr int g = decltype(G)::value, h = g & 1;
        if (g + 1 < NG) request(g + 1, h ^ 1);
        __builtin_amdgcn_sched_barrier(0);
        const u4 (&xs)[2] = x[(g * ILV) >> 3];
#pragma unroll
        for (int k = 0; k < ILV; ++k) acc[(g * ILV + k) & 7] = TM_HF(w[h][k][1], xs[0], acc[(g * ILV + k) & 7]);
#pragma unroll
        for (int k = 0; k < ILV; ++k) acc[(g * ILV + k) & 7] = TM_HF(w[h][k][0], xs[1], acc[(g * ILV + k) & 7]);
#pragma unroll
        for (int k = 0; k < ILV; ++k) acc[(g * ILV + k) & 7] = TM_HF(w[h][k][0], xs[0], acc[(g * ILV + k) & 7]);
        __builtin_amdgcn_sched_barrier(0);
        ride(G);
        __builtin_amdgcn_sched_barrier(0);
    });
#undef TM_HF
}
template <bool DEC, bool OFF32, bool PROF = false>
__global__ __launch_bounds__(512, 2) void msg8_wave_kernel(MsgArgsB a, unsigned long long *prof = nullptr) {
    unsigned t_last = 0, t_acc[8] = {};
    auto mark = [&](int k) {
#ifndef TM_MSG_PROF_NOMARKS
#define TM_MSG_PROF_NOMARKS 0
#endif
        if constexpr (PROF && !TM_MSG_PROF_NOMARKS) {
            __builtin_amdgcn_sched_barrier(0);
            const unsigned t = (unsigned)__builtin_readcyclecounter();
            if (k >= 0) t_acc[k] += t - t_last;
            t_last = t;
        }
    };
    __shared__ __attribute__((aligned(16))) char sW[2 * TM_WIMG_BYTES];
    __shared__ __attribute__((aligned(16))) float s_g0[8][TM_H];
    __shared__ __attribute__((aligned(16))) float s_b2[TM_H];
    const int tid = tm_tid(), lane = tid & 63, wv = tid >> 6, n = lane & 15, q = lane >> 4;
    for (int o = tid * 16; o < TM_WIMG_BYTES; o += 512 * 16) {
        *reinterpret_cast<u4 *>(sW + o) = *reinterpret_cast<const u4 *>(a.imgp1 + o);
        *reinterpret_cast<u4 *>(sW + TM_WIMG_BYTES + o) = *reinterpret_cast<const u4 *>(a.imgp2 + o);
    }
    if (tid < TM_H / 4) st4(&s_b2[4 * tid], ld4(a.b2 + 4 * tid));
    __syncthreads();
    const char *wl1 = sW + 16 * lane, *wl2 = sW + TM_WIMG_BYTES + 16 * lane;
    float *g0s = s_g0[wv];

    const TileRange tr = xcd_tile_range(a.T);
#ifndef TM_MSG_WAVE_OLD_16TH
#define TM_MSG_WAVE_OLD_16TH 11
#endif
    const int n_wg = tr.begin < tr.end ? (tr.end - tr.begin + tr.step - 1) / tr.step : 0;
    const int wvs = tm_wave(tid), simd = wvs & 3;
    const int m_simd = (n_wg - simd + 3) / 4;
    const int n_old = (m_simd * TM_MSG_WAVE_OLD_16TH + 8) / 16;
    const int t0 = wvs < 4 ? 0 : n_old, nt = wvs < 4 ? n_old : m_simd - n_old;
    auto res_at = [&](int t) { return __builtin_amdgcn_readfirstlane(tr.begin + (simd + 4 * (t0 + t)) * tr.step); };
    int t_res = 0;
    if (nt <= 0) return;
    int i = res_at(0);
    const unsigned uq = 4u * (unsigned)q;
    const unsigned eoff = (unsigned)(n * TM_H) + uq;

    auto idx_of = [&](int ii, int bb) { return (a.E_idx + ((size_t)__builtin_amdgcn_readfirstlane(ii) * TM_KS + 16 * __builtin_amdgcn_readfirstlane(bb)))[(unsigned)n]; };
    f4 e_n[8], g_n[8];
    float mk_n = 1.f;
    struct BlockAddr { unsigned goff; const float *pj; const float *src; unsigned jj; };
    auto block_addr = [&](int ii, int bb, int j) {
        const int jj = j < 0 ? ii : j;
        BlockAddr r;
        r.jj = (unsigned)jj;
        r.goff = (unsigned)jj * 256u + (128u + uq);
        r.pj = a.P + (size_t)jj * 256 + 128 + uq;
        r.src = a.hE + ((size_t)__builtin_amdgcn_readfirstlane(ii) * TM_KS + 16 * __builtin_amdgcn_readfirstlane(bb)) * TM_H;
        return r;
    };
    auto issue_piece = [&](const BlockAddr &ad, auto G) {
        constexpr int g = decltype(G)::value;
        if constexpr (g < 8) {
            if constexpr (OFF32) g_n[g] = ld4(a.P + (ad.goff + 16u * g));
            else g_n[g] = ld4(ad.pj + 16 * g);
        } else {
            if (g == 8 && !DEC) mk_n = a.mask[ad.jj];
            e_n[g - 8] = ld4(ad.src + (eoff + 16u * (g - 8)));
        }
    };
    auto issue_block = [&](int ii, int bb, int j) {
        const BlockAddr ad = block_addr(ii, bb, j);
        static_for<0, 16>([&](auto G) { issue_piece(ad, G); });
    };
    f4 g0_n = f4{0.f, 0.f, 0.f, 0.f};
    float mi_n = 0.f;
    auto issue_self = [&](int ii) {
        if (lane < 32) g0_n = ld4(a.P + (size_t)__builtin_amdgcn_readfirstlane(ii) * 256 + 4 * lane);
        mi_n = (a.mask + __builtin_amdgcn_readfirstlane(ii))[0];
    };

    int j_cur = idx_of(i, 0), j_nxt = idx_of(i, 1);
    issue_block(i, 0, j_cur);
    issue_self(i);
    u4 xn[4][2];
#pragma unroll
    for (int c = 0; c < 4; ++c) split_pair(e_n[2 * c], e_n[2 * c + 1], xn[c]);
    f4 sum[8];
    float mi = 0.f, cnt = 0.f;
    mark(-1);
    unsigned long long c_begin = 0, w_begin = 0;
    if (PROF) { c_begin = __builtin_readcyclecounter(); w_begin = wall_clock64(); }
    for (;;) {
        if (lane < 32) st4(g0s + 4 * lane, g0_n);
        mi = mi_n;
        cnt = 0.f;
#pragma unroll
        for (int cb = 0; cb < 8; ++cb) sum[cb] = f4{0.f, 0.f, 0.f, 0.f};
        __builtin_amdgcn_fence(__ATOMIC_RELEASE, "wavefront");
        __builtin_amdgcn_wave_barrier();
        const bool more = t_res + 1 < nt;
        const int inx = more ? res_at(t_res + 1) : i;
#pragma unroll 1
        for (int b = 0; b < 3; ++b) {
            u4 x[4][2];
            f4 acc[8];
#pragma unroll
            for (int c = 0; c < 4; ++c) { x[c][0] = xn[c][0]; x[c][1] = xn[c][1]; }
#pragma unroll
            for (int cb = 0; cb < 8; ++cb) acc[cb] = DEC ? g_n[cb] : g_n[cb] + ld4(g0s + 16 * cb + uq);
#pragma unroll
            for (int c = 0; c < 4; ++c) { asm volatile("" : "+v"(x[c][0]), "+v"(x[c][1])); }
#pragma unroll
            for (int cb = 0; cb < 8; ++cb) touch(acc[cb]);
            mark(0);
            const float ma = j_cur < 0 ? 0.f : (DEC ? 1.f : mi * mk_n);
            const bool last_b = b == 2;
            const bool has1 = !last_b || more;
            const int i1 = has1 ? (last_b ? inx : i) : i, b1 = has1 ? (last_b ? 0 : b + 1) : b;
            const BlockAddr ad1 = block_addr(i1, b1, has1 ? j_nxt : j_cur);
            mark(1);
            mma_wave_lds(wl1, x, acc, [&](auto G) { issue_piece(ad1, G); });
            if (last_b) issue_self(i1);
            {
                const bool last_b1 = b1 == 2;
                const int i2 = last_b1 ? inx : i1, b2 = last_b1 ? 0 : b1 + 1;
                const bool has2 = has1 && (!last_b1 || more);
                j_cur = j_nxt;
                j_nxt = idx_of(has2 ? i2 : i1, has2 ? b2 : b1);
            }
            mark(2);
#pragma unroll
            for (int c = 0; c < 4; ++c) {
                f4 v0 = acc[2 * c], v1 = acc[2 * c + 1];
                if (DEC) {
                    v0 = ld4(g0s + 32 * c + uq) + mi * v0;
                    v1 = ld4(g0s + 32 * c + 16 + uq) + mi * v1;
                }
                split_pair(gelu4(v0), gelu4(v1), x[c]);
            }
#pragma unroll
            for (int cb = 0; cb < 8; ++cb) acc[cb] = ld4(s_b2 + 16 * cb + uq);
            mark(3);
            mma_wave_lds(wl2, x, acc, [&](auto G) {
                constexpr int g = decltype(G)::value;
                if constexpr (g % 3 == 0 && g >= 3 && g <= 12) split_pair(e_n[2 * (g / 3 - 1)], e_n[2 * (g / 3 - 1) + 1], xn[g / 3 - 1]);
            });
            mark(4);
#pragma unroll
            for (int cb = 0; cb < 8; ++cb) {
                const f4 g = gelu4(acc[cb]);
                sum[cb] = f4{__builtin_fmaf(g.x, ma, sum[cb].x), __builtin_fmaf(g.y, ma, sum[cb].y), __builtin_fmaf(g.z, ma, sum[cb].z), __builtin_fmaf(g.w, ma, sum[cb].w)};
            }
            cnt += ma;
            mark(5);
        }
#define TM_ROW_SCAN(x)                                                                                  \
        x += __int_as_float(__builtin_amdgcn_update_dpp(0, __float_as_int(x), 0x111, 0xf, 0xf, true));  \
        x += __int_as_float(__builtin_amdgcn_update_dpp(0, __float_as_int(x), 0x112, 0xf, 0xf, true));  \
        x += __int_as_float(__builtin_amdgcn_update_dpp(0, __float_as_int(x), 0x114, 0xf, 0xf, true));  \
        x += __int_as_float(__builtin_amdgcn_update_dpp(0, __float_as_int(x), 0x118, 0xf, 0xf, true));
#pragma unroll
        for (int cb = 0; cb < 8; ++cb) {
            f4 t = sum[cb];
#pragma unroll
            for (int k = 0; k < 4; ++k) { float v = t[k]; TM_ROW_SCAN(v) t[k] = v; }
            if (n == 15) st4(g0s + 16 * cb + uq, t);
        }
        __builtin_amdgcn_fence(__ATOMIC_RELEASE, "wavefront");
        __builtin_amdgcn_wave_barrier();
        if (lane < 32) st4(a.Ssum + (size_t)__builtin_amdgcn_readfirstlane(i) * TM_H + 4 * lane, ld4(g0s + 4 * lane));
        TM_ROW_SCAN(cnt)
#undef TM_ROW_SCAN
        if (lane == 15) a.cnt[i] = cnt;
        mark(6);
        if (!more) break;
        ++t_res;
        i = inx;
    }
    if (PROF && tm_bid() == 0 && tm_tid() == (TM_PROF_TID & ~63)) {
#pragma unroll
        for (int k = 0; k < 8; ++k) prof[k] = t_acc[k];
        prof[8] = __builtin_readcyclecounter() - c_begin;
        prof[9] = wall_clock64() - w_begin;
    }
    if (PROF && (tm_bid() == 0 || tm_bid() == (int)gridDim.x - 1) && (tm_tid() & 63) == 0)
        prof[(tm_bid() == 0 ? 16 : 24) + (tm_tid() >> 6)] = __builtin_readcyclecounter() - c_begin;
}

int launch_msg_split(int mode, const MsgW &m, const float *P, const float *hE, const int32_t *E_idx, const float *mask, int64_t T,
                     float *Ssum, float *cnt, hipStream_t st) {
    const bool h2 = mode == TM_MM_F16X2, dec = m.dec;
    MsgArgsB a{m.W1e, m.ld1, m.W2, m.b2, P, hE, E_idx, mask, Ssum, cnt, (int)T, m.img.w1, m.img.w2, m.img.p1, m.img.p2, 0};
    if (h2 && !(a.imgp1 && a.imgp2))
        return tm_set_error(TMPNN_E_INVALID, "msg_split: f16x2 handle without the K-permuted fragment images of W1e / W2");
    const int64_t cap = tm_num_cus();
    const bool off32 = T < ((int64_t)1 << 22);
    static const int wave_min = TM_DBG_INT("TMPNN_MSG_WAVE_MIN", TM_MSG_WAVE_MIN);
    int64_t Tw = 0;
    if (h2 && cap % 8 == 0) {
        const int64_t q = T / (8 * cap);
        if (q >= (wave_min > 0 ? wave_min : 1)) Tw = q * 8 * cap;
        else if (wave_min == 0 && T > 0) Tw = T;
    }
    if (Tw > 0) {
        a.T = (int)Tw;
#ifdef TMPNN_DEBUG_BUILD
        static const bool wprof = TM_DBG_FLAG("TMPNN_MSG_PROF", false);
        if (wprof && dec) {
            static unsigned long long *d_prof = nullptr;
            if (!d_prof) (void)hipMalloc(&d_prof, 32 * sizeof(unsigned long long));
            (void)hipMemsetAsync(d_prof, 0, 32 * sizeof(unsigned long long), st);
            msg8_wave_kernel<true, false, true><<<(int)cap, 512, 0, st>>>(a, d_prof);
            unsigned long long h[32];
            (void)hipMemcpy(h, d_prof, sizeof(h), hipMemcpyDeviceToHost);
            fprintf(stderr, "dec_msg wave phases (cycles, one wavefront of wg 0, all its blocks): operands %llu requests %llu gemm1 %llu gelu+split %llu gemm2 %llu gelu+mask %llu ksum+store %llu; loop %llu cycles in %llu ticks of 100 MHz = %.3f GHz\n",
                    h[0], h[1], h[2], h[3], h[4], h[5], h[6], h[8], h[9], h[9] ? h[8] / (h[9] * 10.0) : 0.0);
            fprintf(stderr, "dec_msg wave loops (cycles, the eight wavefronts of wg 0): %llu %llu %llu %llu | %llu %llu %llu %llu; of the last wg: %llu %llu %llu %llu | %llu %llu %llu %llu\n",
                    h[16], h[17], h[18], h[19], h[20], h[21], h[22], h[23], h[24], h[25], h[26], h[27], h[28], h[29], h[30], h[31]);
        } else
#endif
        if (off32) {
            if (dec) msg8_wave_kernel<true, true><<<(int)cap, 512, 0, st>>>(a);
            else msg8_wave_kernel<false, true><<<(int)cap, 512, 0, st>>>(a);
        } else if (dec) msg8_wave_kernel<true, false><<<(int)cap, 512, 0, st>>>(a);
        else msg8_wave_kernel<false, false><<<(int)cap, 512, 0, st>>>(a);
        if (Tw == T) return tm_check_launch(dec ? "dec_msg_wave" : "enc_msg_wave");
        a.i0 = (int)Tw;
        a.T = (int)(T - Tw);
    }
    const int grid = (int)(a.T < cap ? a.T : cap);
    if (mode == TM_MM_BF16X3) {
        if (off32) {
            if (dec) msg8_rp_kernel<SplitBF3, true, false, true><<<grid, 512, 0, st>>>(a);
            else msg8_rp_kernel<SplitBF3, false, false, true><<<grid, 512, 0, st>>>(a);
        } else if (dec) msg8_rp_kernel<SplitBF3, true><<<grid, 512, 0, st>>>(a);
        else msg8_rp_kernel<SplitBF3, false><<<grid, 512, 0, st>>>(a);
    } else {
#ifdef TMPNN_DEBUG_BUILD
        static const bool prof = TM_DBG_FLAG("TMPNN_MSG_PROF", false);
#else
        constexpr bool prof = false;
#endif
        if (prof && dec && Tw == 0) {
#ifdef TMPNN_DEBUG_BUILD
            static unsigned long long *d_prof = nullptr;
            if (!d_prof) (void)hipMalloc(&d_prof, 16 * sizeof(unsigned long long));
            (void)hipMemsetAsync(d_prof, 0, 16 * sizeof(unsigned long long), st);
            msg8_rp_kernel<SplitH2, true, true, false><<<grid, 512, 0, st>>>(a, d_prof);
            unsigned long long h[16];
            (void)hipMemcpy(h, d_prof, sizeof(h), hipMemcpyDeviceToHost);
            fprintf(stderr, "dec_msg phases (cycles, wg 0): fetch+gemm1 %llu gelu+split %llu bar %llu split_tile+gather %llu gemm2 %llu gelu+mask %llu bar %llu ksum+store %llu\n",
                    h[0], h[1], h[2], h[3], h[4], h[5], h[6], h[7]);
#endif
        } else if (off32) {
            if (dec) msg8_rp_kernel<SplitH2, true, false, true><<<grid, 512, 0, st>>>(a);
            else msg8_rp_kernel<SplitH2, false, false, true><<<grid, 512, 0, st>>>(a);
        } else if (dec) msg8_rp_kernel<SplitH2, true><<<grid, 512, 0, st>>>(a);
        else msg8_rp_kernel<SplitH2, false><<<grid, 512, 0, st>>>(a);
    }
    return tm_check_launch(dec ? "dec_msg_split" : "enc_msg_split");
}
```

### thermompnn_amd/csrc/tmpnn_split.h

```cpp
#pragma once
#include <type_traits>

#include "tmpnn_common.h"

typedef __bf16 bf8 __attribute__((ext_vector_type(8)));
typedef __bf16 bf2 __attribute__((ext_vector_type(2)));
typedef _Float16 h8 __attribute__((ext_vector_type(8)));
typedef _Float16 h2 __attribute__((ext_vector_type(2)));
typedef unsigned int u2 __attribute__((ext_vector_type(2)));
typedef unsigned int u4 __attribute__((ext_vector_type(4)));

#define TM_EDGE_PF 2
#define TM_MSG_PF 3
#define TM_NODE_PF 3
#define TM_NODE_DEEP_D 2
#define TM_NODE_DEEP_PF 2
#ifndef TM_PROF_TID
#define TM_PROF_TID 0
#endif
#define SPLIT_PLANE_BYTES (TM_TILE * TM_H * 2)

template <int I, int N, typename F>
__device__ __forceinline__ void static_for(F &&f) {
    if constexpr (I < N) {
        f(std::integral_constant<int, I>{});
        static_for<I + 1, N>(f);
    }
}

struct SplitBF3 {
    static constexpr int NP = 3;
    static constexpr bool EXACT = true;
    static __device__ __forceinline__ void split2(f2 x, unsigned (&p)[3]) {
        const bf2 h = __builtin_convertvector(x, bf2);
        const f2 r1 = x - __builtin_convertvector(h, f2);
        const bf2 m = __builtin_convertvector(r1, bf2);
        const f2 r2 = r1 - __builtin_convertvector(m, f2);
        const bf2 l = __builtin_convertvector(r2, bf2);
        p[0] = __builtin_bit_cast(unsigned, h);
        p[1] = __builtin_bit_cast(unsigned, m);
        p[2] = __builtin_bit_cast(unsigned, l);
    }
    static __device__ __forceinline__ f2 join2(const unsigned (&p)[3]) {
        const f2 h = __builtin_convertvector(__builtin_bit_cast(bf2, p[0]), f2);
        const f2 m = __builtin_convertvector(__builtin_bit_cast(bf2, p[1]), f2);
        const f2 l = __builtin_convertvector(__builtin_bit_cast(bf2, p[2]), f2);
        return (h + m) + l;
    }
    static __device__ __forceinline__ void mma(const u4 (&w)[3], const u4 (&x)[3], f4 &acc, f4 &lo) {
#define TM_BF(a, b, c) __builtin_amdgcn_mfma_f32_16x16x32_bf16(__builtin_bit_cast(bf8, a), __builtin_bit_cast(bf8, b), c, 0, 0, 0)
        lo = TM_BF(w[2], x[0], lo);
        lo = TM_BF(w[0], x[2], lo);
        lo = TM_BF(w[1], x[1], lo);
        lo = TM_BF(w[1], x[0], lo);
        lo = TM_BF(w[0], x[1], lo);
        acc = TM_BF(w[0], x[0], acc);
#undef TM_BF
    }
    static __device__ __forceinline__ f4 fold(f4 acc, f4 lo) { return acc + lo; }
};

struct SplitH2 {
    static constexpr int NP = 2;
    static constexpr bool EXACT = false;
    static __device__ __forceinline__ void split2(f2 x, unsigned (&p)[2]) {
        const h2 h = __builtin_convertvector(x, h2);
        p[0] = __builtin_bit_cast(unsigned, h);
#if TM_ABL_NOSPLIT
        p[1] = 0u;
        return;
#endif
        const f2 r = x - __builtin_convertvector(h, f2);
        const h2 l = __builtin_convertvector(r, h2);
        p[1] = __builtin_bit_cast(unsigned, l);
    }
    static __device__ __forceinline__ f2 join2(const unsigned (&p)[2]) {
        const f2 h = __builtin_convertvector(__builtin_bit_cast(h2, p[0]), f2);
        const f2 l = __builtin_convertvector(__builtin_bit_cast(h2, p[1]), f2);
        return h + l;
    }
    static __device__ __forceinline__ void mma(const u4 (&w)[2], const u4 (&x)[2], f4 &acc, f4 &lo) {
#define TM_HF(a, b, c) __builtin_amdgcn_mfma_f32_16x16x32_f16(__builtin_bit_cast(h8, a), __builtin_bit_cast(h8, b), c, 0, 0, 0)
        acc = TM_HF(w[1], x[0], acc);
        acc = TM_HF(w[0], x[1], acc);
        acc = TM_HF(w[0], x[0], acc);
#undef TM_HF
    }
    static __device__ __forceinline__ f4 fold(f4 acc, f4 lo) { return acc; }
};

template <int ROWS = TM_TILE, int ROWB = 256>
__device__ __forceinline__ int plane_off4(int p, int row, int c4) {
    return p * (ROWS * ROWB) + row * ROWB + ((((c4 >> 1) ^ (row & 15)) << 4) | ((c4 & 1) << 3));
}
template <int ROWS = TM_TILE, int ROWB = 256, bool SWZ = true>
__device__ __forceinline__ int plane_off8(int p, int row, int c16) {
    return p * (ROWS * ROWB) + row * ROWB + ((SWZ ? (c16 ^ (row & 15)) : c16) << 4);
}

template <typename SP, int ROWS = TM_TILE, int ROWB = 256>
__device__ __forceinline__ void store_split(char *tile, int row, int c4, f4 v) {
    unsigned a[SP::NP], b[SP::NP];
    SP::split2(f2{v.x, v.y}, a);
    SP::split2(f2{v.z, v.w}, b);
#pragma unroll
    for (int p = 0; p < SP::NP; ++p) *reinterpret_cast<u2 *>(tile + plane_off4<ROWS, ROWB>(p, row, c4)) = u2{a[p], b[p]};
}
template <typename SP, int ROWS = TM_TILE, int ROWB = 256>
__device__ __forceinline__ f4 load_joined(const char *tile, int row, int c4) {
    unsigned a[SP::NP], b[SP::NP];
#pragma unroll
    for (int p = 0; p < SP::NP; ++p) {
        const u2 w = *reinterpret_cast<const u2 *>(tile + plane_off4<ROWS, ROWB>(p, row, c4));
        a[p] = w.x;
        b[p] = w.y;
    }
    const f2 lo = SP::join2(a), hi = SP::join2(b);
    return f4{lo.x, lo.y, hi.x, hi.y};
}

template <typename SP>
struct WFragS { u4 p[SP::NP]; };

template <typename SP, int NK32, bool PERM = false>
__device__ __forceinline__ void load_wfrag_split(const float *__restrict__ W, int ld, int n0, int k0, int k_valid,
                                                 WFragS<SP> (&wf)[NK32], int lane, int k_wrap = 0) {
    const float *src = W + (size_t)(n0 + (lane & 15)) * ld + k0 + (PERM ? 4 : 8) * (lane >> 4);
#pragma unroll
    for (int c = 0; c < NK32; ++c) {
        unsigned w[4][SP::NP];
#pragma unroll
        for (int half = 0; half < 2; ++half) {
            const int k = 32 * c + (PERM ? 4 : 8) * (lane >> 4) + (PERM ? 16 : 4) * half;
            const f4 v = k < k_valid ? ld4(src + 32 * c + (PERM ? 16 : 4) * half) : k < k_valid + k_wrap ? ld4(src + 32 * c + 4 * half - ld) : f4{0.f, 0.f, 0.f, 0.f};
            SP::split2(f2{v.x, v.y}, w[2 * half]);
            SP::split2(f2{v.z, v.w}, w[2 * half + 1]);
        }
#pragma unroll
        for (int p = 0; p < SP::NP; ++p) wf[c].p[p] = u4{w[0][p], w[1][p], w[2][p], w[3][p]};
    }
}

template <typename SP, int NK32, int NCB, int NRB = 3, int ROWS = TM_TILE, int ROWB = 256, int NKTOT = NK32, int C0 = 0,
          bool SWZ = true, int PF = 0>
__device__ __forceinline__ void mma_tile_split(const char *tile, const WFragS<SP> (&w)[NCB][NKTOT], f4 (&acc)[NRB][NCB], int lane) {
#if TM_ABL_NOMFMA
    return;
#endif
    const int m = lane & 15, q = lane >> 4;
    f4 lo[NRB][NCB];
#pragma unroll
    for (int rb = 0; rb < NRB; ++rb)
#pragma unroll
        for (int cb = 0; cb < NCB; ++cb) lo[rb][cb] = f4{0.f, 0.f, 0.f, 0.f};
    if constexpr (PF > 0) {
        constexpr int NS = NK32 * NRB, NB = PF + 1;
        u4 x[NB][SP::NP];
#pragma unroll
        for (int s = 0; s < PF && s < NS; ++s)
#pragma unroll
            for (int p = 0; p < SP::NP; ++p)
                x[s][p] = *reinterpret_cast<const u4 *>(tile + plane_off8<ROWS, ROWB, SWZ>(p, 16 * (s % NRB) + m, 4 * (s / NRB) + q));
#pragma unroll
        for (int s = 0; s < NS; ++s) {
            if (s + PF < NS) {
                const int sn = s + PF;
#pragma unroll
                for (int p = 0; p < SP::NP; ++p)
                    x[sn % NB][p] = *reinterpret_cast<const u4 *>(tile + plane_off8<ROWS, ROWB, SWZ>(p, 16 * (sn % NRB) + m, 4 * (sn / NRB) + q));
            }
            __builtin_amdgcn_sched_barrier(0);
#pragma unroll
            for (int cb = 0; cb < NCB; ++cb) SP::mma(w[cb][C0 + s / NRB].p, x[s % NB], acc[s % NRB][cb], lo[s % NRB][cb]);
            __builtin_amdgcn_sched_barrier(0);
        }
    } else if constexpr (PF < 0) {
#pragma unroll
        for (int c = 0; c < NK32; ++c) {
            u4 x[NRB][SP::NP];
#pragma unroll
            for (int rb = 0; rb < NRB; ++rb)
#pragma unroll
                for (int p = 0; p < SP::NP; ++p)
                    x[rb][p] = *reinterpret_cast<const u4 *>(tile + plane_off8<ROWS, ROWB, SWZ>(p, 16 * rb + m, 4 * c + q));
            __builtin_amdgcn_sched_barrier(0);
#pragma unroll
            for (int rb = 0; rb < NRB; ++rb)
#pragma unroll
                for (int cb = 0; cb < NCB; ++cb) SP::mma(w[cb][C0 + c].p, x[rb], acc[rb][cb], lo[rb][cb]);
            __builtin_amdgcn_sched_barrier(0);
        }
    } else {
#pragma unroll
        for (int c = 0; c < NK32; ++c) {
#pragma unroll
            for (int rb = 0; rb < NRB; ++rb) {
                u4 x[SP::NP];
#pragma unroll
                for (int p = 0; p < SP::NP; ++p)
                    x[p] = *reinterpret_cast<const u4 *>(tile + plane_off8<ROWS, ROWB, SWZ>(p, 16 * rb + m, 4 * c + q));
#pragma unroll
                for (int cb = 0; cb < NCB; ++cb) SP::mma(w[cb][C0 + c].p, x, acc[rb][cb], lo[rb][cb]);
            }
        }
    }
#pragma unroll
    for (int rb = 0; rb < NRB; ++rb)
#pragma unroll
        for (int cb = 0; cb < NCB; ++cb) acc[rb][cb] = SP::fold(acc[rb][cb], lo[rb][cb]);
}

template <typename SP, int NK32, int NRB, int PF, int ROWS = TM_TILE, typename R>
__device__ __forceinline__ void mma_tile_split_ride(const char *tile, const WFragS<SP> (&w)[1][NK32], f4 (&acc)[NRB][1], int lane, R &&ride) {
    constexpr int NS = NK32 * NRB, NB = PF + 1;
#if TM_ABL_NOMFMA
    static_for<0, NS>([&](auto S) { ride(S); });
    return;
#endif
    const int m = lane & 15, q = lane >> 4;
    f4 lo[NRB][1];
#pragma unroll
    for (int rb = 0; rb < NRB; ++rb) lo[rb][0] = f4{0.f, 0.f, 0.f, 0.f};
    u4 x[NB][SP::NP];
#pragma unroll
    for (int s = 0; s < PF && s < NS; ++s)
#pragma unroll
        for (int p = 0; p < SP::NP; ++p)
            x[s][p] = *reinterpret_cast<const u4 *>(tile + plane_off8<ROWS, 256, true>(p, 16 * (s % NRB) + m, 4 * (s / NRB) + q));
    static_for<0, NS>([&](auto S) {
        constexpr int s = decltype(S)::value;
        if constexpr (s + PF < NS) {
            constexpr int sn = s + PF;
#pragma unroll
            for (int p = 0; p < SP::NP; ++p)
                x[sn % NB][p] = *reinterpret_cast<const u4 *>(tile + plane_off8<ROWS, 256, true>(p, 16 * (sn % NRB) + m, 4 * (sn / NRB) + q));
        }
        __builtin_amdgcn_sched_barrier(0);
        SP::mma(w[0][s / NRB].p, x[s % NB], acc[s % NRB][0], lo[s % NRB][0]);
        __builtin_amdgcn_sched_barrier(0);
        ride(S);
        __builtin_amdgcn_sched_barrier(0);
    });
#pragma unroll
    for (int rb = 0; rb < NRB; ++rb) acc[rb][0] = SP::fold(acc[rb][0], lo[rb][0]);
}

template <typename SP, int NK32, int NCB, int ROWS = TM_TILE, int ROWB = 256>
__device__ __forceinline__ void mma_rb_split(const char *tile, int rb, const WFragS<SP> (&w)[NCB][NK32], f4 (&acc)[NCB], int lane) {
    const int m = lane & 15, q = lane >> 4;
    f4 lo[NCB];
#pragma unroll
    for (int cb = 0; cb < NCB; ++cb) lo[cb] = f4{0.f, 0.f, 0.f, 0.f};
#pragma unroll
    for (int c = 0; c < NK32; ++c) {
        u4 x[SP::NP];
#pragma unroll
        for (int p = 0; p < SP::NP; ++p)
            x[p] = *reinterpret_cast<const u4 *>(tile + plane_off8<ROWS, ROWB>(p, 16 * rb + m, 4 * c + q));
#pragma unroll
        for (int cb = 0; cb < NCB; ++cb) SP::mma(w[cb][c].p, x, acc[cb], lo[cb]);
    }
#pragma unroll
    for (int cb = 0; cb < NCB; ++cb) acc[cb] = SP::fold(acc[cb], lo[cb]);
}

__device__ __forceinline__ void row_stats_partial1b(const f4 v, float *stat_slot, int q) {
    float mean = (v.x + v.y + v.z + v.w) * 0.25f;
    const f4 d = v - mean;
    float m2 = d.x * d.x + d.y * d.y + d.z * d.z + d.w * d.w;
    {
        const auto pm = __builtin_amdgcn_permlane16_swap(__float_as_uint(mean), __float_as_uint(mean), false, false);
        const auto p2 = __builtin_amdgcn_permlane16_swap(__float_as_uint(m2), __float_as_uint(m2), false, false);
        const float ma = __uint_as_float(pm[0]), mb = __uint_as_float(pm[1]);
        const float delta = mb - ma;
        mean = 0.5f * (ma + mb);
        m2 = __uint_as_float(p2[0]) + __uint_as_float(p2[1]) + delta * delta * 2.0f;
    }
    {
        const auto pm = __builtin_amdgcn_permlane32_swap(__float_as_uint(mean), __float_as_uint(mean), false, false);
        const auto p2 = __builtin_amdgcn_permlane32_swap(__float_as_uint(m2), __float_as_uint(m2), false, false);
        const float ma = __uint_as_float(pm[0]), mb = __uint_as_float(pm[1]);
        const float delta = mb - ma;
        mean = 0.5f * (ma + mb);
        m2 = __uint_as_float(p2[0]) + __uint_as_float(p2[1]) + delta * delta * 4.0f;
    }
    if (q == 0) *reinterpret_cast<f2 *>(stat_slot) = f2{mean, m2};
}
#define TM_STAT8_LD 20
__device__ __forceinline__ void row_stats_finish8b(const float *stat_row, float &mean, float &rstd) {
    f4 p[4];
#pragma unroll
    for (int k = 0; k < 4; ++k) p[k] = ld4(stat_row + 4 * k);
    mean = 0.125f * (p[0].x + p[0].z + p[1].x + p[1].z + p[2].x + p[2].z + p[3].x + p[3].z);
    float m2 = 0.f, dd = 0.f;
#pragma unroll
    for (int k = 0; k < 4; ++k) {
        const float d0 = p[k].x - mean, d1 = p[k].z - mean;
        m2 += p[k].y + p[k].w;
        dd += d0 * d0 + d1 * d1;
    }
    rstd = __builtin_amdgcn_rsqf((m2 + 16.f * dd) * (1.0f / 128.0f) + 1e-5f);
}

#define TM_STAT_LD 18
__device__ __forceinline__ float swap_add16(float x) {
    const auto p = __builtin_amdgcn_permlane16_swap(__float_as_uint(x), __float_as_uint(x), false, false);
    return __uint_as_float(p[0]) + __uint_as_float(p[1]);
}
__device__ __forceinline__ float swap_add32(float x) {
    const auto p = __builtin_amdgcn_permlane32_swap(__float_as_uint(x), __float_as_uint(x), false, false);
    return __uint_as_float(p[0]) + __uint_as_float(p[1]);
}
__device__ __forceinline__ void row_stats_partial16(const f4 v, float *stat_slot, int q) {
    const float s = swap_add32(swap_add16((v.x + v.y) + (v.z + v.w)));
    const float mean = s * 0.0625f;
    const f4 d = v - mean;
    const float m2 = swap_add32(swap_add16(__builtin_fmaf(d.w, d.w, __builtin_fmaf(d.z, d.z, __builtin_fmaf(d.y, d.y, d.x * d.x)))));
    if (q == 0) *reinterpret_cast<f2 *>(stat_slot) = f2{mean, m2};
}
__device__ __forceinline__ float allreduce8_dpp(float x) {
    x += __int_as_float(__builtin_amdgcn_update_dpp(0, __float_as_int(x), 0xB1, 0xf, 0xf, true));
    x += __int_as_float(__builtin_amdgcn_update_dpp(0, __float_as_int(x), 0x4E, 0xf, 0xf, true));
    x += __int_as_float(__builtin_amdgcn_update_dpp(0, __float_as_int(x), 0x141, 0xf, 0xf, true));
    return x;
}
__device__ __forceinline__ void row_stats_finish8d(const float *stat_row, int lane, float &mean, float &rstd) {
    const f2 p = *reinterpret_cast<const f2 *>(stat_row + 2 * (lane & 7));
    mean = allreduce8_dpp(p.x) * 0.125f;
    const float d = p.x - mean;
    const float m2 = allreduce8_dpp(__builtin_fmaf(16.f * d, d, p.y));
    rstd = __builtin_amdgcn_rsqf(__builtin_fmaf(m2, 1.0f / 128.0f, 1e-5f));
}

__device__ __forceinline__ int perm_c4(int c4) { return (c4 & ~7) | ((c4 & 3) << 1) | ((c4 >> 2) & 1); }

template <typename SP, bool PERM = false>
__device__ __forceinline__ void load_wfrag_auto(const char *img, const float *__restrict__ W, int ld, int wv, int lane,
                                                WFragS<SP> (&wf)[4]) {
    if (img != nullptr && SP::NP == 2) {
        const char *p = img + (size_t)wv * 8192 + lane * 16;
#pragma unroll
        for (int c = 0; c < 4; ++c) {
            wf[c].p[0] = *reinterpret_cast<const u4 *>(p + 2048 * c);
            wf[c].p[1] = *reinterpret_cast<const u4 *>(p + 2048 * c + 1024);
        }
    } else {
        load_wfrag_split<SP, 4, PERM>(W, ld, 16 * wv, 0, TM_H, wf, lane);
    }
}

struct EdgeArgsB {
    const float *W11e, *W12, *b12, *W13, *b13, *g3, *be3, *P;
    float *hE;
    const int32_t *E_idx;
    int T;
    const char *img11, *img12, *img13;
};

struct MsgArgsB {
    const float *W1e; int ld1;
    const float *W2, *b2, *P;
    const float *hE;
    const int32_t *E_idx;
    const float *mask;
    float *Ssum, *cnt;
    int T;
    const char *img1, *img2;
    const char *imgp1, *imgp2;
    int i0;
};

__device__ __forceinline__ void split_pair(const f4 a, const f4 b, u4 (&x)[2]) {
    unsigned p0[2], p1[2], p2[2], p3[2];
    SplitH2::split2(f2{a.x, a.y}, p0);
    SplitH2::split2(f2{a.z, a.w}, p1);
    SplitH2::split2(f2{b.x, b.y}, p2);
    SplitH2::split2(f2{b.z, b.w}, p3);
    x[0] = u4{p0[0], p1[0], p2[0], p3[0]};
    x[1] = u4{p0[1], p1[1], p2[1], p3[1]};
}
```

Baseline: 123.0 million preds/s.

## Store final encoder edge features as pre-split f16x2 fragment image for decoder

When the decoder message pass uses the wave kernel in f16x2 mode and edge-message fusion is off, the last encoder edge kernel now writes hE directly as the split f16 hi/lo fragment image the decoder consumes. The decoder message kernels then load that image instead of re-splitting fp32 edges on every one of the three decoder layers. This removes repeated split_pair work and reorganizes the per-row LayerNorm store in the edge kernel. In exchange the hE buffer layout changes for the decoder, with new template variants and a layout dependency across kernels.

```diff
diff --git a/thermompnn_amd/csrc/tmpnn_api.hip b/thermompnn_amd/csrc/tmpnn_api.hip
--- a/thermompnn_amd/csrc/tmpnn_api.hip
+++ b/thermompnn_amd/csrc/tmpnn_api.hip
@@ -383,7 +383,7 @@
 
 static int run_enc_layer(const tmpnn_weights *w, int l, float *hV, float *hE, const int32_t *E_idx, const float *mask,
                          int64_t T, const LayerWs &ws, bool have_P, bool have_msg, const NodeProj *next, const MsgW *then,
-                         hipStream_t st) {
+                         hipStream_t st, bool dec_img = false) {
     const EncW &e = w->enc[l];
     if (!have_P) {
         const NodeProj mp = enc_msg_proj(w, l, ws.P);
@@ -393,26 +393,26 @@
     const NodeProj ep = enc_edge_proj(w, l, ws.P2);
     TRY(launch_node_update(w->mode, e.node, hV, ws.Ssum, ws.cnt, mask, T, hV, &ep, next, st));
     if (then) return launch_edge_msg_fused(e.edge, ws.P2, hE, E_idx, *then, ws.P, mask, T, ws.Ssum, ws.cnt, st);
-    return launch_enc_edge(w->mode, e.edge, ws.P2, hE, E_idx, T, st);
+    return launch_enc_edge(w->mode, e.edge, ws.P2, hE, E_idx, T, st, dec_img);
 }
 
 static int run_dec_layer(const tmpnn_weights *w, int l, const float *hV_in, float *hV_out, const float *hE,
                          const int32_t *E_idx, const int32_t *S, const float *mask, int64_t T, const LayerWs &ws,
                          bool have_P, bool have_msg, const NodeProj *next, hipStream_t st, const HeadArgs *head = nullptr,
-                         bool *head_ran = nullptr) {
+                         bool *head_ran = nullptr, bool dec_img = false) {
     const DecW &d = w->dec[l];
     if (!have_P) {
         const NodeProj mp = dec_msg_proj(w, l, ws.P, S);
         TRY(launch_node_proj(hV_in, mp, T, st));
     }
-    if (!have_msg) TRY(launch_msg(w->mode, d.msg, ws.P, hE, E_idx, mask, T, ws.Ssum, ws.cnt, st));
+    if (!have_msg) TRY(launch_msg(w->mode, d.msg, ws.P, hE, E_idx, mask, T, ws.Ssum, ws.cnt, st, dec_img));
     return launch_node_update(w->mode, d.node, hV_in, ws.Ssum, ws.cnt, mask, T, hV_out, next, nullptr, st, head, head_ran);
 }
 
 static int run_encoder(const tmpnn_weights *w, const float *X, const float *mask, const int32_t *residue_idx, const int32_t *chain_enc,
                        const int32_t *offsets, int n_proteins, int64_t T, int max_len, int K, const LayerWs &ws, int32_t *E_idx,
                        float *D_nb, float *hE, float *hV, const int32_t *S, float *P_dec0, int32_t *status_opt, bool *dec_msg0_done,
-                       hipStream_t st) {
+                       hipStream_t st, bool *hE_dec_img = nullptr) {
     static const bool fuse_small = TM_DBG_FLAG("TMPNN_FUSE_SMALL", true);
     const KnnInit kinit{hV, ws.P, w->enc[0].msg_proj.spec.ba, status_opt};
     if (fuse_small && max_len <= 256 && featurize_fusable(w->mode, T)) {
@@ -424,10 +424,13 @@
     }
     const bool fused = fuse_small && edge_msg_fusable(w->mode, T);
     *dec_msg0_done = fused && S;
+    static const bool dec_img_on = TM_DBG_FLAG("TMPNN_DEC_IMG", true);
+    const bool dec_img = dec_img_on && hE_dec_img && S && w->mode == TM_MM_F16X2 && !fused && msg_takes_wave(w->mode, T);
+    if (hE_dec_img) *hE_dec_img = dec_img;
     for (int l = 0; l < 3; ++l) {
         const NodeProj next = l < 2 ? enc_msg_proj(w, l + 1, ws.P) : dec_msg_proj(w, 0, P_dec0, S);
         const MsgW *then = !fused ? nullptr : l < 2 ? &w->enc[l + 1].msg : S ? &w->dec[0].msg : nullptr;
-        TRY(run_enc_layer(w, l, hV, hE, E_idx, mask, T, ws, true, fused && l > 0, &next, then, st));
+        TRY(run_enc_layer(w, l, hV, hE, E_idx, mask, T, ws, true, fused && l > 0, &next, then, st, dec_img && l == 2));
     }
     return TMPNN_OK;
 }
@@ -625,15 +628,16 @@
 
     bool dec_msg0_done = false;
     bool head_done = false;
+    bool dec_img = false;
     TRY(run_encoder(w, X, mask, residue_idx, chain_enc, offsets, n_proteins, T, max_len, K, ws, E_idx, D_nb, hE, hV[0], S, ws.P,
-                    status_opt, &dec_msg0_done, st));
+                    status_opt, &dec_msg0_done, st, &dec_img));
     for (int l = 0; l < 3; ++l) {
         const NodeProj next = dec_msg_proj(w, l < 2 ? l + 1 : 2, ws.P, S);
         HeadArgs ha;
         const bool with_head = dec_msg0_done && l == 2 && ddg && node_head_fusable(w->mode, T);
         if (with_head) TRY(tm_head_args(ha, w, hV[3], hV[2], S, T, ddg, nullptr, status_opt, E_idx));
         TRY(run_dec_layer(w, l, hV[l], hV[l + 1], hE, E_idx, S, mask, T, ws, true, dec_msg0_done && l == 0, l < 2 ? &next : nullptr, st,
-                          with_head ? &ha : nullptr, with_head ? &head_done : nullptr));
+                          with_head ? &ha : nullptr, with_head ? &head_done : nullptr, dec_img));
     }
     if (ddg && !head_done) TRY(launch_head(w, hV[3], hV[2], S, T, ddg, nullptr, status_opt, st, E_idx));
     if (log_probs_opt) TRY(launch_log_probs(w, hV[3], T, log_probs_opt, status_opt, st, ddg ? nullptr : E_idx));
diff --git a/thermompnn_amd/csrc/tmpnn_edge.hip b/thermompnn_amd/csrc/tmpnn_edge.hip
--- a/thermompnn_amd/csrc/tmpnn_edge.hip
+++ b/thermompnn_amd/csrc/tmpnn_edge.hip
@@ -6,8 +6,9 @@
 #include "tmpnn_split.h"
 #include "tmpnn_internal.h"
 
-template <typename SP, bool PROF = false, bool OFF32 = false>
+template <typename SP, bool PROF = false, bool OFF32 = false, bool IMG = false>
 __global__ __launch_bounds__(512, 2) void enc_edge8_rp_kernel(EdgeArgsB a, unsigned long long *prof = nullptr) {
+    static_assert(!IMG || SP::NP == 2, "the decoder image is the f16x2 B operand");
     unsigned t_last = 0, t_acc[11] = {};
     auto mark = [&](int k) {
         if constexpr (PROF) {
@@ -22,7 +23,7 @@
     __shared__ __attribute__((aligned(16))) char tX[TILEB];
     __shared__ __attribute__((aligned(16))) char tY[TILEB];
     __shared__ __attribute__((aligned(16))) float tO[TM_TILE * TM_H];
-    __shared__ __attribute__((aligned(16))) float s_par[SP::EXACT ? 4 : 1][TM_H];
+    __shared__ __attribute__((aligned(16))) float s_par[SP::EXACT ? 4 : IMG ? 2 : 1][TM_H];
     __shared__ __attribute__((aligned(16))) float s_stat[TM_TILE][TM_STAT_LD];
     __shared__ int s_idx[2][TM_TILE];
     const int tid = tm_tid(), lane = tid & 63, wv = tid >> 6, m = lane & 15, q = lane >> 4;
@@ -44,11 +45,17 @@
     constexpr int EPF = SP::EXACT ? 1 : TM_EDGE_PF;
     const f4 z4p = f4{0.f, 0.f, 0.f, 0.f};
     f4 b12r = z4p, b13r = z4p, g4r = z4p, be4r = z4p;
+    const int wu = tm_wave(tid);
+    const int irow = 16 * (wu < 4 ? wu >> 1 : 2) + m;
     if constexpr (SP::EXACT) {
         if (tid < 128) st4(&s_par[tid >> 5][4 * (tid & 31)], ld4((tid < 32 ? a.b12 : tid < 64 ? a.b13 : tid < 96 ? a.g3 : a.be3) + 4 * (tid & 31)));
     } else {
         b12r = ld4(a.b12 + ncol); b13r = ld4(a.b13 + ncol);
-        g4r = ld4(a.g3 + 4 * c32); be4r = ld4(a.be3 + 4 * c32);
+        if constexpr (IMG) {
+            if (tid < 64) st4(&s_par[tid >> 5][4 * c32], ld4((tid < 32 ? a.g3 : a.be3) + 4 * c32));
+        } else {
+            g4r = ld4(a.g3 + 4 * c32); be4r = ld4(a.be3 + 4 * c32);
+        }
     }
     auto par = [&](int k, int col, const f4 &reg) -> f4 { if constexpr (SP::EXACT) return ld4(&s_par[k][col]); else return reg; };
 
@@ -160,7 +167,7 @@
         }
         bool okr[3];
 #pragma unroll
-        for (int it = 0; it < 3; ++it) okr[it] = s_idx[cur][6 * wv + 2 * it + (lane >> 5)] >= 0;
+        for (int it = 0; it < 3; ++it) okr[it] = s_idx[cur][IMG ? irow : 6 * wv + 2 * it + (lane >> 5)] >= 0;
         mark(7);
         __syncthreads();
         mark(8);
@@ -168,6 +175,39 @@
         touch(gai);
 #pragma unroll
         for (int rb = 0; rb < 3; ++rb) touch(gcj[rb]);
+        auto ln4 = [](const f4 x4, const f4 g4, const f4 be4, float mean, float rstd) {
+            const f2 s01 = f2{g4.x, g4.y} * rstd, s23 = f2{g4.z, g4.w} * rstd;
+            const f2 t01 = __builtin_elementwise_fma(f2{-mean, -mean}, s01, f2{be4.x, be4.y});
+            const f2 t23 = __builtin_elementwise_fma(f2{-mean, -mean}, s23, f2{be4.z, be4.w});
+            const f2 y01 = __builtin_elementwise_fma(f2{x4.x, x4.y}, s01, t01), y23 = __builtin_elementwise_fma(f2{x4.z, x4.w}, s23, t23);
+            return f4{y01.x, y01.y, y23.x, y23.y};
+        };
+        if constexpr (IMG) {
+            const int bI = wu < 4 ? wu >> 1 : 2;
+            float mean = 0.f, rstd = 1.f;
+#if !TM_ABL_NOLN
+            row_stats_finish8q(&s_stat[irow][0], q, mean, rstd);
+#endif
+            const bool some_empty = __builtin_amdgcn_ballot_w64(!okr[0]) != 0;
+#pragma unroll
+            for (int u = 0; u < 2; ++u) {
+                if (u == 1 && wu >= 4) break;
+                const int cI = wu < 4 ? 2 * (wu & 1) + u : wu - 4, col = 32 * cI + 4 * q;
+                f4 ya = ln4(ld4(tO + chunk_off(irow, 8 * cI + q)), ld4(&s_par[0][col]), ld4(&s_par[1][col]), mean, rstd);
+                f4 yb = ln4(ld4(tO + chunk_off(irow, 8 * cI + 4 + q)), ld4(&s_par[0][col + 16]), ld4(&s_par[1][col + 16]), mean, rstd);
+                if (some_empty) {
+                    asm volatile("");
+                    const f4 z4 = f4{0.f, 0.f, 0.f, 0.f};
+                    ya = okr[0] ? ya : z4;
+                    yb = okr[0] ? yb : z4;
+                }
+                u4 x[2];
+                split_pair(ya, yb, x);
+                char *dst = reinterpret_cast<char *>(tile_g) + dec_img_off(bI, cI, 0) + 16 * lane;
+                *reinterpret_cast<u4 *>(dst) = x[0];
+                *reinterpret_cast<u4 *>(dst + 1024) = x[1];
+            }
+        } else {
 #pragma unroll
         for (int it = 0; it < 3; ++it) {
             const int row = 6 * wv + 2 * it + (lane >> 5);
@@ -176,13 +216,9 @@
             row_stats_finish8d(&s_stat[row][0], lane, mean, rstd);
 #endif
             const f4 x4 = ld4(tO + chunk_off(row, c32));
-            const f4 g4 = par(2, 4 * c32, g4r), be4 = par(3, 4 * c32, be4r);
-            const f2 s01 = f2{g4.x, g4.y} * rstd, s23 = f2{g4.z, g4.w} * rstd;
-            const f2 t01 = __builtin_elementwise_fma(f2{-mean, -mean}, s01, f2{be4.x, be4.y});
-            const f2 t23 = __builtin_elementwise_fma(f2{-mean, -mean}, s23, f2{be4.z, be4.w});
-            const f2 y01 = __builtin_elementwise_fma(f2{x4.x, x4.y}, s01, t01), y23 = __builtin_elementwise_fma(f2{x4.z, x4.w}, s23, t23);
-            const f4 y = f4{y01.x, y01.y, y23.x, y23.y};
+            const f4 y = ln4(x4, par(2, 4 * c32, g4r), par(3, 4 * c32, be4r), mean, rstd);
             st4(tile_g + (soff + 2 * it * TM_H), okr[it] ? y : f4{0.f, 0.f, 0.f, 0.f});
+        }
         }
         cur ^= 1;
         mark(9);
@@ -196,8 +232,9 @@
     }
 }
 
-int launch_enc_edge_split(int mode, const EdgeW &e, const float *P, float *hE, const int32_t *E_idx, int64_t T, hipStream_t st) {
+int launch_enc_edge_split(int mode, const EdgeW &e, const float *P, float *hE, const int32_t *E_idx, int64_t T, hipStream_t st, bool dec_img) {
     const bool h2 = mode == TM_MM_F16X2;
+    if (dec_img && !h2) return tm_set_error(TMPNN_E_INVALID, "enc_edge_split: the decoder image is an f16x2 form");
     EdgeArgsB a{e.W11e, e.W12, e.b12, e.W13, e.b13, e.n3w, e.n3b, P, hE, E_idx, (int)T, e.img.w11, e.img.w12, e.img.w13};
     if (h2 && !(a.img11 && a.img12 && a.img13))
         return tm_set_error(TMPNN_E_INVALID, "enc_edge_split: f16x2 handle without the fragment images of W11e / W12 / W13");
@@ -218,16 +255,20 @@
             static unsigned long long *d_prof = nullptr;
             if (!d_prof) (void)hipMalloc(&d_prof, 16 * sizeof(unsigned long long));
             (void)hipMemsetAsync(d_prof, 0, 16 * sizeof(unsigned long long), st);
-            enc_edge8_rp_kernel<SplitH2, true, false><<<grid, 512, 0, st>>>(a, d_prof);
+            if (dec_img) enc_edge8_rp_kernel<SplitH2, true, false, true><<<grid, 512, 0, st>>>(a, d_prof);
+            else enc_edge8_rp_kernel<SplitH2, true, false><<<grid, 512, 0, st>>>(a, d_prof);
             unsigned long long h[16];
             (void)hipMemcpy(h, d_prof, sizeof(h), hipMemcpyDeviceToHost);
             const long long tiles0 = T >= 8 * cap ? (T / 8 + cap / 8 - 1) / (cap / 8) : (T + cap - 1) / cap;
-            fprintf(stderr, "enc_edge phases (cycles, wg 0): gemm1 %llu gelu+split %llu bar %llu gather+gemm2 %llu gelu+split %llu bar %llu gemm3 %llu resid+stats %llu bar %llu split+ln+store %llu bar %llu; loop %llu cycles in %llu ticks of 100 MHz = %.3f GHz, %lld tiles = %.0f cycles per tile\n",
-                    h[0], h[1], h[2], h[3], h[4], h[5], h[6], h[7], h[8], h[9], h[10], h[11], h[12], h[12] ? h[11] / (h[12] * 10.0) : 0.0,
+            fprintf(stderr, "enc_edge%s phases (cycles, wg 0): gemm1 %llu gelu+split %llu bar %llu gather+gemm2 %llu gelu+split %llu bar %llu gemm3 %llu resid+stats %llu bar %llu split+ln+store %llu bar %llu; loop %llu cycles in %llu ticks of 100 MHz = %.3f GHz, %lld tiles = %.0f cycles per tile\n",
+                    dec_img ? " (decoder image)" : "", h[0], h[1], h[2], h[3], h[4], h[5], h[6], h[7], h[8], h[9], h[10], h[11], h[12], h[12] ? h[11] / (h[12] * 10.0) : 0.0,
                     tiles0, tiles0 ? (double)h[11] / tiles0 : 0.0);
 #endif
         } else if (T < ((int64_t)1 << 22)) {
-            enc_edge8_rp_kernel<SplitH2, false, true><<<grid, 512, 0, st>>>(a);
+            if (dec_img) enc_edge8_rp_kernel<SplitH2, false, true, true><<<grid, 512, 0, st>>>(a);
+            else enc_edge8_rp_kernel<SplitH2, false, true><<<grid, 512, 0, st>>>(a);
+        } else if (dec_img) {
+            enc_edge8_rp_kernel<SplitH2, false, false, true><<<grid, 512, 0, st>>>(a);
         } else {
             enc_edge8_rp_kernel<SplitH2><<<grid, 512, 0, st>>>(a);
         }
diff --git a/thermompnn_amd/csrc/tmpnn_internal.h b/thermompnn_amd/csrc/tmpnn_internal.h
--- a/thermompnn_amd/csrc/tmpnn_internal.h
+++ b/thermompnn_amd/csrc/tmpnn_internal.h
@@ -77,7 +77,7 @@
 int launch_gather_edges(const float *edges, const int64_t *idx, int B, int N, int K, int C, float *out, hipStream_t st);
 
 int launch_msg(int mode, const MsgW &m, const float *P, const float *hE, const int32_t *E_idx, const float *mask, int64_t T,
-               float *Ssum, float *cnt, hipStream_t st);
+               float *Ssum, float *cnt, hipStream_t st, bool dec_img = false);
 struct NodeArgs {
     const float *W3, *b3, *n1w, *n1b, *Win, *bin, *Wout, *bout, *n2w, *n2b;
     const float *h_in, *Ssum, *cnt, *mask;
@@ -93,7 +93,7 @@
 int launch_node_update(int mode, const NodeW &n, const float *h_in, const float *Ssum, const float *cnt, const float *mask, int64_t T,
                        float *h_out, const NodeProj *p0, const NodeProj *p1, hipStream_t st, const HeadArgs *head = nullptr,
                        bool *head_ran = nullptr);
-int launch_enc_edge(int mode, const EdgeW &e, const float *P, float *hE, const int32_t *E_idx, int64_t T, hipStream_t st);
+int launch_enc_edge(int mode, const EdgeW &e, const float *P, float *hE, const int32_t *E_idx, int64_t T, hipStream_t st, bool dec_img = false);
 
 int launch_head(const tmpnn_weights *w, const float *hA, const float *hB, const int32_t *S, int64_t T, float *ddg,
                 float *z_opt, int32_t *status, hipStream_t st, const int32_t *maxlen_probe = nullptr);
@@ -120,9 +120,11 @@
 
 int launch_clock_probe(int blocks, int iters, unsigned long long *out, float *sink, hipStream_t st);
 int launch_clock_monitor(int iters, unsigned long long *out, hipStream_t st);
-int launch_enc_edge_split(int mode, const EdgeW &e, const float *P, float *hE, const int32_t *E_idx, int64_t T, hipStream_t st);
+int launch_enc_edge_split(int mode, const EdgeW &e, const float *P, float *hE, const int32_t *E_idx, int64_t T, hipStream_t st,
+                          bool dec_img = false);
 int launch_msg_split(int mode, const MsgW &m, const float *P, const float *hE, const int32_t *E_idx, const float *mask, int64_t T,
-                     float *Ssum, float *cnt, hipStream_t st);
+                     float *Ssum, float *cnt, hipStream_t st, bool dec_img = false);
+bool msg_takes_wave(int mode, int64_t T);
 int launch_gemm_probe(int mode, const float *X, const float *W, float *Y, int64_t T, int reps, hipStream_t st);
 bool edge_msg_fusable(int mode, int64_t T);
 int launch_edge_msg_fused(const EdgeW &e, const float *P_edge, float *hE, const int32_t *E_idx, const MsgW &m, const float *P_msg,
diff --git a/thermompnn_amd/csrc/tmpnn_layers.hip b/thermompnn_amd/csrc/tmpnn_layers.hip
--- a/thermompnn_amd/csrc/tmpnn_layers.hip
+++ b/thermompnn_amd/csrc/tmpnn_layers.hip
@@ -445,11 +445,12 @@
 }
 
 int launch_msg(int mode, const MsgW &m, const float *P, const float *hE, const int32_t *E_idx, const float *mask, int64_t T,
-               float *Ssum, float *cnt, hipStream_t st) {
+               float *Ssum, float *cnt, hipStream_t st, bool dec_img) {
     const bool dec = m.dec;
+    if (dec_img && mode != TM_MM_F16X2) return tm_set_error(TMPNN_E_INVALID, "msg: the decoder image is an f16x2 form");
     tm_prof_begin(dec ? "dec_msg" : "enc_msg", st);
     if (mode != TM_MM_FP32) {
-        const int rc = launch_msg_split(mode, m, P, hE, E_idx, mask, T, Ssum, cnt, st);
+        const int rc = launch_msg_split(mode, m, P, hE, E_idx, mask, T, Ssum, cnt, st, dec_img);
         tm_prof_end(st);
         return rc;
     }
@@ -460,10 +461,11 @@
     return tm_check_launch(dec ? "dec_msg" : "enc_msg");
 }
 
-int launch_enc_edge(int mode, const EdgeW &e, const float *P, float *hE, const int32_t *E_idx, int64_t T, hipStream_t st) {
+int launch_enc_edge(int mode, const EdgeW &e, const float *P, float *hE, const int32_t *E_idx, int64_t T, hipStream_t st, bool dec_img) {
+    if (dec_img && mode != TM_MM_F16X2) return tm_set_error(TMPNN_E_INVALID, "enc_edge: the decoder image is an f16x2 form");
     tm_prof_begin("enc_edge", st);
     if (mode != TM_MM_FP32) {
-        const int rc = launch_enc_edge_split(mode, e, P, hE, E_idx, T, st);
+        const int rc = launch_enc_edge_split(mode, e, P, hE, E_idx, T, st, dec_img);
         tm_prof_end(st);
         return rc;
     }
diff --git a/thermompnn_amd/csrc/tmpnn_msg.hip b/thermompnn_amd/csrc/tmpnn_msg.hip
--- a/thermompnn_amd/csrc/tmpnn_msg.hip
+++ b/thermompnn_amd/csrc/tmpnn_msg.hip
@@ -6,8 +6,9 @@
 #include "tmpnn_split.h"
 #include "tmpnn_internal.h"
 
-template <typename SP, bool DEC, bool PROF = false, bool OFF32 = false>
+template <typename SP, bool DEC, bool PROF = false, bool OFF32 = false, bool IMG = false>
 __global__ __launch_bounds__(512, 2) void msg8_rp_kernel(MsgArgsB a, unsigned long long *prof = nullptr) {
+    static_assert(!IMG || (DEC && SP::NP == 2), "the decoder image is the f16x2 B operand of the decoder's message pass");
     unsigned long long t_last = 0;
     auto mark = [&](int k) {
         if (PROF && tm_bid() == 0 && tm_tid() == TM_PROF_TID) {
@@ -52,16 +53,20 @@
     };
     const int prow = 6 * wv + (lane >> 5), pc = lane & 31;
     const int pcs = PERM ? perm_c4(pc) : pc;
-    const unsigned eoff = (unsigned)(prow * TM_H + 4 * pc);
+    const unsigned eoff = IMG ? 4u * (unsigned)tid : (unsigned)(prow * TM_H + 4 * pc);
+    constexpr unsigned ESTEP = IMG ? 2048u : 2u * TM_H;
     auto fetch_into = [&](f4 (&dst)[3], int ii) {
         const float *src = a.hE + (size_t)__builtin_amdgcn_readfirstlane(ii) * (TM_KS * TM_H);
 #pragma unroll
-        for (int it = 0; it < 3; ++it) dst[it] = ld4(src + (eoff + 2 * it * TM_H));
+        for (int it = 0; it < 3; ++it) dst[it] = ld4(src + (eoff + it * ESTEP));
     };
     auto fetch_tile = [&](int ii) { fetch_into(e_nxt, ii); };
     auto split_tile = [&]() {
 #pragma unroll
-        for (int it = 0; it < 3; ++it) store_split<SP>(tE, prow + 2 * it, pcs, e_nxt[it]);
+        for (int it = 0; it < 3; ++it) {
+            if constexpr (IMG) *reinterpret_cast<f4 *>(tE + plane_off8(wv & 1, 16 * it + m, 4 * (wv >> 1) + q)) = e_nxt[it];
+            else store_split<SP>(tE, prow + 2 * it, pcs, e_nxt[it]);
+        }
     };
 
     TileRange tr = xcd_tile_range(a.T);
@@ -123,7 +128,7 @@
                 else gj[s - 1] = ld4(a.P + (size_t)j * 256 + 128 + ncol);
             }
 #if !TM_ABL_NOLOAD
-            if constexpr (s >= 5 && s <= 9 && (s & 1)) e_nxt[(s - 5) >> 1] = ld4(src3 + (eoff + 2 * ((s - 5) >> 1) * TM_H));
+            if constexpr (s >= 5 && s <= 9 && (s & 1)) e_nxt[(s - 5) >> 1] = ld4(src3 + (eoff + ((s - 5) >> 1) * ESTEP));
 #endif
         });
         mark(4);
@@ -212,8 +217,9 @@
     });
 #undef TM_HF
 }
-template <bool DEC, bool OFF32, bool PROF = false>
+template <bool DEC, bool OFF32, bool PROF = false, bool IMG = false>
 __global__ __launch_bounds__(512, 2) void msg8_wave_kernel(MsgArgsB a, unsigned long long *prof = nullptr) {
+    static_assert(!IMG || DEC, "the decoder image is read by the decoder's message pass only");
     unsigned t_last = 0, t_acc[8] = {};
     auto mark = [&](int k) {
 #ifndef TM_MSG_PROF_NOMARKS
@@ -253,10 +259,11 @@
     if (nt <= 0) return;
     int i = res_at(0);
     const unsigned uq = 4u * (unsigned)q;
-    const unsigned eoff = (unsigned)(n * TM_H) + uq;
+    const unsigned eoff = IMG ? 4u * (unsigned)lane : (unsigned)(n * TM_H) + uq;
 
     auto idx_of = [&](int ii, int bb) { return (a.E_idx + ((size_t)__builtin_amdgcn_readfirstlane(ii) * TM_KS + 16 * __builtin_amdgcn_readfirstlane(bb)))[(unsigned)n]; };
     f4 e_n[8], g_n[8];
+    u4 xn[4][2];
     float mk_n = 1.f;
     struct BlockAddr { unsigned goff; const float *pj; const float *src; unsigned jj; };
     auto block_addr = [&](int ii, int bb, int j) {
@@ -275,7 +282,8 @@
             else g_n[g] = ld4(ad.pj + 16 * g);
         } else {
             if (g == 8 && !DEC) mk_n = a.mask[ad.jj];
-            e_n[g - 8] = ld4(ad.src + (eoff + 16u * (g - 8)));
+            if constexpr (IMG) xn[(g - 8) >> 1][(g - 8) & 1] = __builtin_bit_cast(u4, ld4(ad.src + (eoff + 256u * (g - 8))));
+            else e_n[g - 8] = ld4(ad.src + (eoff + 16u * (g - 8)));
         }
     };
     auto issue_block = [&](int ii, int bb, int j) {
@@ -292,9 +300,10 @@
     int j_cur = idx_of(i, 0), j_nxt = idx_of(i, 1);
     issue_block(i, 0, j_cur);
     issue_self(i);
-    u4 xn[4][2];
-#pragma unroll
-    for (int c = 0; c < 4; ++c) split_pair(e_n[2 * c], e_n[2 * c + 1], xn[c]);
+    if constexpr (!IMG) {
+#pragma unroll
+        for (int c = 0; c < 4; ++c) split_pair(e_n[2 * c], e_n[2 * c + 1], xn[c]);
+    }
     f4 sum[8];
     float mi = 0.f, cnt = 0.f;
     mark(-1);
@@ -353,7 +362,7 @@
             mark(3);
             mma_wave_lds(wl2, x, acc, [&](auto G) {
                 constexpr int g = decltype(G)::value;
-                if constexpr (g % 3 == 0 && g >= 3 && g <= 12) split_pair(e_n[2 * (g / 3 - 1)], e_n[2 * (g / 3 - 1) + 1], xn[g / 3 - 1]);
+                if constexpr (!IMG && g % 3 == 0 && g >= 3 && g <= 12) split_pair(e_n[2 * (g / 3 - 1)], e_n[2 * (g / 3 - 1) + 1], xn[g / 3 - 1]);
             });
             mark(4);
 #pragma unroll
@@ -397,21 +406,26 @@
         prof[(tm_bid() == 0 ? 16 : 24) + (tm_tid() >> 6)] = __builtin_readcyclecounter() - c_begin;
 }
 
+static int64_t msg_wave_part(int64_t T) {
+    const int64_t cap = tm_num_cus();
+    static const int wave_min = TM_DBG_INT("TMPNN_MSG_WAVE_MIN", TM_MSG_WAVE_MIN);
+    if (cap % 8 != 0) return 0;
+    const int64_t q = T / (8 * cap);
+    if (q >= (wave_min > 0 ? wave_min : 1)) return q * 8 * cap;
+    return wave_min == 0 && T > 0 ? T : 0;
+}
+bool msg_takes_wave(int mode, int64_t T) { return mode == TM_MM_F16X2 && msg_wave_part(T) > 0; }
+
 int launch_msg_split(int mode, const MsgW &m, const float *P, const float *hE, const int32_t *E_idx, const float *mask, int64_t T,
-                     float *Ssum, float *cnt, hipStream_t st) {
+                     float *Ssum, float *cnt, hipStream_t st, bool dec_img) {
     const bool h2 = mode == TM_MM_F16X2, dec = m.dec;
+    if (dec_img && !(h2 && dec)) return tm_set_error(TMPNN_E_INVALID, "msg_split: the decoder image is read by the f16x2 decoder pass only");
     MsgArgsB a{m.W1e, m.ld1, m.W2, m.b2, P, hE, E_idx, mask, Ssum, cnt, (int)T, m.img.w1, m.img.w2, m.img.p1, m.img.p2, 0};
     if (h2 && !(a.imgp1 && a.imgp2))
         return tm_set_error(TMPNN_E_INVALID, "msg_split: f16x2 handle without the K-permuted fragment images of W1e / W2");
     const int64_t cap = tm_num_cus();
     const bool off32 = T < ((int64_t)1 << 22);
-    static const int wave_min = TM_DBG_INT("TMPNN_MSG_WAVE_MIN", TM_MSG_WAVE_MIN);
-    int64_t Tw = 0;
-    if (h2 && cap % 8 == 0) {
-        const int64_t q = T / (8 * cap);
-        if (q >= (wave_min > 0 ? wave_min : 1)) Tw = q * 8 * cap;
-        else if (wave_min == 0 && T > 0) Tw = T;
-    }
+    const int64_t Tw = h2 ? msg_wave_part(T) : 0;
     if (Tw > 0) {
         a.T = (int)Tw;
 #ifdef TMPNN_DEBUG_BUILD
@@ -420,7 +434,8 @@
             static unsigned long long *d_prof = nullptr;
             if (!d_prof) (void)hipMalloc(&d_prof, 32 * sizeof(unsigned long long));
             (void)hipMemsetAsync(d_prof, 0, 32 * sizeof(unsigned long long), st);
-            msg8_wave_kernel<true, false, true><<<(int)cap, 512, 0, st>>>(a, d_prof);
+            if (dec_img) msg8_wave_kernel<true, false, true, true><<<(int)cap, 512, 0, st>>>(a, d_prof);
+            else msg8_wave_kernel<true, false, true><<<(int)cap, 512, 0, st>>>(a, d_prof);
             unsigned long long h[32];
             (void)hipMemcpy(h, d_prof, sizeof(h), hipMemcpyDeviceToHost);
             fprintf(stderr, "dec_msg wave phases (cycles, one wavefront of wg 0, all its blocks): operands %llu requests %llu gemm1 %llu gelu+split %llu gemm2 %llu gelu+mask %llu ksum+store %llu; loop %llu cycles in %llu ticks of 100 MHz = %.3f GHz\n",
@@ -429,7 +444,10 @@
                     h[16], h[17], h[18], h[19], h[20], h[21], h[22], h[23], h[24], h[25], h[26], h[27], h[28], h[29], h[30], h[31]);
         } else
 #endif
-        if (off32) {
+        if (dec_img) {
+            if (off32) msg8_wave_kernel<true, true, false, true><<<(int)cap, 512, 0, st>>>(a);
+            else msg8_wave_kernel<true, false, false, true><<<(int)cap, 512, 0, st>>>(a);
+        } else if (off32) {
             if (dec) msg8_wave_kernel<true, true><<<(int)cap, 512, 0, st>>>(a);
             else msg8_wave_kernel<false, true><<<(int)cap, 512, 0, st>>>(a);
         } else if (dec) msg8_wave_kernel<true, false><<<(int)cap, 512, 0, st>>>(a);
@@ -451,7 +469,10 @@
 #else
         constexpr bool prof = false;
 #endif
-        if (prof && dec && Tw == 0) {
+        if (dec_img) {
+            if (off32) msg8_rp_kernel<SplitH2, true, false, true, true><<<grid, 512, 0, st>>>(a);
+            else msg8_rp_kernel<SplitH2, true, false, false, true><<<grid, 512, 0, st>>>(a);
+        } else if (prof && dec && Tw == 0) {
 #ifdef TMPNN_DEBUG_BUILD
             static unsigned long long *d_prof = nullptr;
             if (!d_prof) (void)hipMalloc(&d_prof, 16 * sizeof(unsigned long long));
diff --git a/thermompnn_amd/csrc/tmpnn_split.h b/thermompnn_amd/csrc/tmpnn_split.h
--- a/thermompnn_amd/csrc/tmpnn_split.h
+++ b/thermompnn_amd/csrc/tmpnn_split.h
@@ -332,7 +332,16 @@
     rstd = __builtin_amdgcn_rsqf(__builtin_fmaf(m2, 1.0f / 128.0f, 1e-5f));
 }
 
+__device__ __forceinline__ void row_stats_finish8q(const float *stat_row, int q, float &mean, float &rstd) {
+    const f2 p0 = *reinterpret_cast<const f2 *>(stat_row + 4 * q), p1 = *reinterpret_cast<const f2 *>(stat_row + 4 * q + 2);
+    mean = swap_add32(swap_add16(p0.x + p1.x)) * 0.125f;
+    const float d0 = p0.x - mean, d1 = p1.x - mean;
+    const float m2 = swap_add32(swap_add16(__builtin_fmaf(16.f * d0, d0, p0.y) + __builtin_fmaf(16.f * d1, d1, p1.y)));
+    rstd = __builtin_amdgcn_rsqf(__builtin_fmaf(m2, 1.0f / 128.0f, 1e-5f));
+}
+
 __device__ __forceinline__ int perm_c4(int c4) { return (c4 & ~7) | ((c4 & 3) << 1) | ((c4 >> 2) & 1); }
+__device__ __forceinline__ int dec_img_off(int b, int c, int p) { return ((b * 4 + c) * 2 + p) * 1024; }
 
 template <typename SP, bool PERM = false>
 __device__ __forceinline__ void load_wfrag_auto(const char *img, const float *__restrict__ W, int ld, int wv, int lane,
```

After: 124.6 million preds/s, median of 6. 1.2% higher.
